# iKrishneel/fcn_object_detector

Measured on AMD Instinct MI355X. Metric: frames/sec forward 448x448 @1 GPU; train imgs/sec @1/2/4/8 GPUs, higher is better.
Workload: dtype f32; 1 GPU; configs[1]: single-GPU forward, DetectNet GoogLeNet conv stack + coverage/bbox heads (graph of models/deploy.prototxt), batch=1, 448x448, random-init weights; global_batch=1, parallelism=replicas x1, frames_in_flight=4

## Files before the change

fcn_object_detector_amd/csrc/conv_fwd.hip:

```cpp
#include <cstddef>
#include <algorithm>
#include <mutex>
#include <unordered_map>
#include <type_traits>

#include "common.h"
#include "conv_common.h"

using namespace fcn;

namespace fcn {

const float* zero_page_for_current_device(int* rc) {
    static std::mutex mu;
    static const float* pages[64] = {nullptr};
    int dev = 0;
    *rc = 0;
    if (hipGetDevice(&dev) != hipSuccess || dev < 0 || dev >= 64) {
        *rc = set_err(FCN_E_STATE, "conv: no current device");
        return nullptr;
    }
    std::lock_guard<std::mutex> lock(mu);
    if (!pages[dev]) {
        void* ptr = nullptr;
        hipError_t e = hipMalloc(&ptr, 256);
        if (e == hipSuccess) e = hipMemset(ptr, 0, 256);
        if (e != hipSuccess) {
            *rc = set_err(-(int)e, "conv: zero page allocation failed: %s", hipGetErrorString(e));
            return nullptr;
        }
        pages[dev] = reinterpret_cast<const float*>(ptr);
    }
    return pages[dev];
}

}

namespace {

constexpr int kPoolItemsPerThread = 2;
constexpr int kPoolSmallItems = 128 * 1024;

template <typename T, int NT>
__device__ __forceinline__ void pool_body(const PoolP& q, int wg) {
    constexpr int EPS = 16 / (int)sizeof(T);
    typedef T vec_t __attribute__((ext_vector_type(EPS)));
    const int cg = q.C / EPS;
    const T* x = reinterpret_cast<const T*>(q.x);
    T* y = reinterpret_cast<T*>(q.y);
    const int ipt = q.items <= kPoolSmallItems ? 1 : kPoolItemsPerThread;
#pragma unroll
    for (int it = 0; it < kPoolItemsPerThread; ++it) {
        if (it >= ipt) return;
        const int t = (wg * ipt + it) * NT + (int)threadIdx.x;
        if (t >= q.items) return;
        const int pix = t / cg;
        const int g = t - pix * cg;
        const int row = pix / q.OW;
        const int ox = pix - row * q.OW;
        const int n = row / q.OH;
        const int oy = row - n * q.OH;
        int hs = oy * q.stride - q.pad, ws = ox * q.stride - q.pad;
        const int he = min(hs + q.k, q.H), we = min(ws + q.k, q.W);
        hs = max(hs, 0);
        ws = max(ws, 0);
        const T* xb = x + (size_t)n * q.H * q.W * q.x_cstride + g * EPS;
        vec_t m;
        int mi[EPS];
#pragma unroll
        for (int e = 0; e < EPS; ++e) {
            m[e] = sizeof(T) == 2 ? (T)-65504.f : (T)-3.402823466e+38f;
            mi[e] = -1;
        }
        if (q.k == 3) {
            const int y0 = oy * q.stride - q.pad, x0 = ox * q.stride - q.pad;
            vec_t v[9];
            int id[9];
            bool in[9];
#pragma unroll
            for (int r = 0; r < 3; ++r) {
                const int iy = min(max(y0 + r, 0), q.H - 1);
#pragma unroll
                for (int c = 0; c < 3; ++c) {
                    const int ix = min(max(x0 + c, 0), q.W - 1);
                    in[3 * r + c] = (int)((unsigned)(y0 + r) < (unsigned)q.H) & (int)((unsigned)(x0 + c) < (unsigned)q.W);
                    id[3 * r + c] = iy * q.W + ix;
                    v[3 * r + c] = *(const vec_t*)(xb + (size_t)id[3 * r + c] * q.x_cstride);
                }
            }
#pragma unroll
// ... 817 lines not shown
    }
#endif
}

__device__ __forceinline__ const GroupArgs& group_of(const GroupArgs& a) { return a; }
__device__ __forceinline__ const GroupArgs& group_of(const GroupArgsTail& a) { return a.g; }
#ifdef FCN_EXP_TAIL_NOLDS
constexpr int kTailLdsFloats = 0;
#else
constexpr int kTailLdsFloats = kTailRows * 32 + 4;
#endif

template <typename T, int WTM, int WTN, int WAVES_M, int WAVES_N, int WAVES_K, int BK, int NBUF, bool PF, bool TAIL = false>
__global__ __launch_bounds__((Cfg<WTM, WTN, WAVES_M, WAVES_N, WAVES_K, BK, NBUF, PF>::NT)) void conv_fwd_group(const int nprob, const int te0, const int te1, const int te2,
                                                                                  const int te3, const int te4, const int te5, const int te6,
                                                                                  const int te7, const int pool_wgs, const int snake,
                                                                                  const std::conditional_t<TAIL, GroupArgsTail, GroupArgs> a_) {
    __shared__ __attribute__((aligned(16))) float smem[Cfg<WTM, WTN, WAVES_M, WAVES_N, WAVES_K, BK, NBUF, PF>::LDS_FLOATS + (TAIL ? kTailLdsFloats : 0)];
    const GroupArgs& a = group_of(a_);
    typedef unsigned u32x16 __attribute__((ext_vector_type(16)));
    typedef unsigned u32x8 __attribute__((ext_vector_type(8)));
    typedef const GroupArgs __attribute__((address_space(4))) * karg_ptr;
    static_assert(alignof(GroupArgsTail) == alignof(GroupArgs) && offsetof(GroupArgsTail, g) == 0, "the group leads its tail");
    constexpr size_t kArgsOffset = (11 * sizeof(int) + alignof(GroupArgs) - 1) / alignof(GroupArgs) * alignof(GroupArgs);
    karg_ptr ka = (karg_ptr)((const char __attribute__((address_space(4)))*)__builtin_amdgcn_kernarg_segment_ptr() + kArgsOffset);
    const int head[1 + kMaxGroup] = {nprob, te0, te1, te2, te3, te4, te5, te6, te7};
    static_assert(kMaxGroup == 8, "the tile prefix travels as eight scalar kernel arguments");
    const int pool_first = pool_wgs > 0 ? pool_wgs : 0;
    if ((int)blockIdx.x < pool_first || (pool_wgs < 0 && (int)blockIdx.x >= te7)) {
        const int w = pool_wgs < 0 ? (int)blockIdx.x - te7 : (int)blockIdx.x;
        if (w < a.pool[0].wg_end) pool_body<T, Cfg<WTM, WTN, WAVES_M, WAVES_N, WAVES_K, BK, NBUF, PF>::NT>(a.pool[0], w);
        else pool_body<T, Cfg<WTM, WTN, WAVES_M, WAVES_N, WAVES_K, BK, NBUF, PF>::NT>(a.pool[1], w - a.pool[0].wg_end);
        return;
    }
    int pos = blockIdx.x;
    if (snake > 0) {
        const int sh = snake & 255, rounds = snake >> 8;
        const int r = pos >> sh, j = pos & ((1 << sh) - 1);
        if (r > 0 && r < rounds - 1 && ((rounds - 1 - r) & 1)) pos = (r << sh) + ((1 << sh) - 1 - j);
    }
    int tile = pos - pool_first;
    if (snake == (int)0x80000000) {
        const int x = pos & 7, sl = pos >> 3, q = te7 >> 3, r = te7 & 7;
        tile = x * q + (x < r ? x : r) + sl;
    } else if (snake < 0) {
        tile += snake;
        tile += tile < 0 ? te7 : 0;
    }
    int pi = 0, begin = 0;
#pragma unroll
    for (int i = 0; i < kMaxGroup - 1; ++i) {
        const int end_i = head[1 + i];
        const bool past = i + 1 < nprob && tile >= end_i;
        pi += past ? 1 : 0;
        begin = past ? end_i : begin;
    }
    u32x16 ra, rb;
    u32x8 rc;
    pi = __builtin_amdgcn_readfirstlane(pi);
    begin = __builtin_amdgcn_readfirstlane(begin);
    const ConvP __attribute__((address_space(4)))* pbase = &ka->p[pi];
    asm volatile("s_load_dwordx16 %0, %3, 0x0\n\ts_load_dwordx16 %1, %3, 0x40\n\ts_load_dwordx8 %2, %3, 0x80\n\ts_waitcnt lgkmcnt(0)"
                 : "=&s"(ra), "=&s"(rb), "=&s"(rc)
                 : "s"(pbase)
                 : "memory");
    ConvP prob;
    __builtin_memcpy((char*)&prob, &ra, 64);
    __builtin_memcpy((char*)&prob + 64, &rb, 64);
    __builtin_memcpy((char*)&prob + 128, &rc, 32);
    if constexpr (TAIL) {
        tail_kptr tp = (tail_kptr)((const char __attribute__((address_space(4)))*)ka + offsetof(GroupArgsTail, tail));
        conv_body<T, WTM, WTN, WAVES_M, WAVES_N, WAVES_K, BK, NBUF, PF, true>(prob, tile - begin, smem, tp);
    } else {
        conv_body<T, WTM, WTN, WAVES_M, WAVES_N, WAVES_K, BK, NBUF, PF>(prob, tile - begin, smem);
    }
}

template <typename T, int WTM, int WTN, int WAVES_M, int WAVES_N, int WAVES_K, int BK, int NBUF, bool PF>
__global__ __launch_bounds__((Cfg<WTM, WTN, WAVES_M, WAVES_N, WAVES_K, BK, NBUF, PF>::NT)) void conv_fwd_one(ConvP p) {
    __shared__ __attribute__((aligned(16))) float smem[Cfg<WTM, WTN, WAVES_M, WAVES_N, WAVES_K, BK, NBUF, PF>::LDS_FLOATS];
    conv_body<T, WTM, WTN, WAVES_M, WAVES_N, WAVES_K, BK, NBUF, PF>(p, blockIdx.x, smem);
}

constexpr int kD7Th = 8, kD7Tw = 32;
constexpr int kD7Ph = 2 * kD7Th + 5, kD7Pw = 2 * kD7Tw + 6;
constexpr int kD7RowF = kD7Pw * 3;
constexpr int kD7PatchF = kD7Ph * kD7RowF;
constexpr int kD7WRowF = 22, kD7WPitchF = 7 * kD7WRowF;
constexpr int kD7WOff = (kD7PatchF + 3) / 4 * 4;
constexpr int kD7EpiPitch = 68;
constexpr int kD7StageF = kD7WOff + 64 * kD7WPitchF;
constexpr int kD7EpiF = 4 * 2 * 32 * kD7EpiPitch;
constexpr int kD7LdsBytes = (kD7StageF > kD7EpiF ? kD7StageF : kD7EpiF) * 4;
constexpr int kD7Threads = 256;
static_assert(kD7LdsBytes <= 80 * 1024, "first-layer kernel: two workgroups per CU");

__global__ __launch_bounds__(kD7Threads) void conv_first7_kernel(const ConvP p) {
#if defined(__HIP_DEVICE_COMPILE__)
    __shared__ __attribute__((aligned(16))) float smem[kD7LdsBytes / 4];
    const int tid = threadIdx.x, lane = tid & 63, wave = __builtin_amdgcn_readfirstlane(tid >> 6);
    FCN_STAMP(0);
    const int tiles_x = (p.OW + kD7Tw - 1) / kD7Tw, tiles_y = (p.OH + kD7Th - 1) / kD7Th;
    int t = blockIdx.x;
    const int tx = t % tiles_x;
    t /= tiles_x;
    const int ty = t % tiles_y, n = t / tiles_y;
    const int oy0 = ty * kD7Th, ox0 = tx * kD7Tw;
    const int iy0 = 2 * oy0 - 3, ix0 = 2 * ox0 - 3;
    const v4f zero4 = {0.f, 0.f, 0.f, 0.f};
    constexpr int PI = (kD7Ph * kD7Pw + kD7Threads - 1) / kD7Threads, WI = (64 * 49 + kD7Threads - 1) / kD7Threads;
    v4f px[PI], wv[WI];
    const float* xn = p.x + (size_t)n * p.H * p.W * 4;
#pragma unroll
    for (int i = 0; i < PI; ++i) {
        const int s = tid + kD7Threads * i;
        const int pr = s / kD7Pw, pc = s - pr * kD7Pw;
        const int iy = iy0 + pr, ix = ix0 + pc;
        const bool ok = s < kD7Ph * kD7Pw && (unsigned)iy < (unsigned)p.H && (unsigned)ix < (unsigned)p.W;
        px[i] = ok ? *reinterpret_cast<const v4f*>(xn + ((size_t)iy * p.W + ix) * 4) : zero4;
    }
#pragma unroll
    for (int i = 0; i < WI; ++i) {
        const int tp = tid + kD7Threads * i;
        wv[i] = tp < p.Cout * 49 ? *reinterpret_cast<const v4f*>(p.w + (size_t)tp * 4) : zero4;
    }
#pragma unroll
    for (int i = 0; i < PI; ++i) {
        const int s = tid + kD7Threads * i;
        if (s < kD7Ph * kD7Pw) {
            float* d = smem + s * 3;
            d[0] = px[i][0]; d[1] = px[i][1]; d[2] = px[i][2];
        }
    }
#pragma unroll
    for (int i = 0; i < WI; ++i) {
        const int tp = tid + kD7Threads * i;
        if (tp < 64 * 49) {
            const int co = tp / 49, rq = tp - co * 49;
            const int r = rq / 7, q = rq - r * 7;
            float* d = smem + kD7WOff + co * kD7WPitchF + r * kD7WRowF + q * 3;
            d[0] = wv[i][0]; d[1] = wv[i][1]; d[2] = wv[i][2];
        }
    }
    for (int i = tid; i < 64 * 7; i += kD7Threads) smem[kD7WOff + i * kD7WRowF + 21] = 0.f;
    const int c4 = (lane & 15) * 4;
    const v4f bias_v = (p.bias && c4 < p.Cout) ? *reinterpret_cast<const v4f*>(p.bias + c4) : zero4;
    FCN_STAMP(1);
    const int nl = lane & 31, h = lane >> 5;
    const float* a_base = smem + (4 * wave) * kD7RowF + 6 * nl + h;
    const float* b_base = smem + kD7WOff + nl * kD7WPitchF + h;
    typedef float v16f __attribute__((ext_vector_type(16)));
    v16f acc[2][2];
#pragma unroll
    for (int i = 0; i < 2; ++i)
#pragma unroll
        for (int j = 0; j < 2; ++j)
#pragma unroll
            for (int e = 0; e < 16; ++e) acc[i][j][e] = 0.f;
    __syncthreads();
    FCN_STAMP(2);
    auto frag = [&](const int step, float (&a)[2], float (&b)[2]) {
        const int r = step / 11, j = step - 11 * r;
#pragma unroll
        for (int mt = 0; mt < 2; ++mt) a[mt] = a_base[(2 * mt + r) * kD7RowF + 2 * j];
#pragma unroll
        for (int nt = 0; nt < 2; ++nt) b[nt] = b_base[nt * 32 * kD7WPitchF + r * kD7WRowF + 2 * j];
    };
    float fa[3][2], fb[3][2];
    frag(0, fa[0], fb[0]);
    frag(1, fa[1], fb[1]);
#pragma unroll
    for (int step = 0; step < 77; ++step) {
        if (step + 2 < 77) frag(step + 2, fa[(step + 2) % 3], fb[(step + 2) % 3]);
        __builtin_amdgcn_sched_barrier(0);
#pragma unroll
        for (int mt = 0; mt < 2; ++mt)
#pragma unroll
            for (int nt = 0; nt < 2; ++nt)
                acc[mt][nt] = __builtin_amdgcn_mfma_f32_32x32x2f32(fa[step % 3][mt], fb[step % 3][nt], acc[mt][nt], 0, 0, 0);
    }
    FCN_STAMP(3);
    __syncthreads();
    float* epi = smem + wave * (2 * 32 * kD7EpiPitch);
#pragma unroll
    for (int mt = 0; mt < 2; ++mt)
#pragma unroll
        for (int nt = 0; nt < 2; ++nt)
#pragma unroll
            for (int v = 0; v < 16; ++v) epi[(mt * 32 + (v & 3) + 8 * (v >> 2) + 4 * h) * kD7EpiPitch + nl + 32 * nt] = acc[mt][nt][v];
    asm volatile("s_waitcnt lgkmcnt(0)" ::: "memory");
    __builtin_amdgcn_sched_barrier(0);
    const bool do_relu = (p.flags & FCN_CONV_RELU) != 0;
#pragma unroll
    for (int mt = 0; mt < 2; ++mt) {
        const int oy = oy0 + 2 * wave + mt;
        float* yrow = p.y + ((size_t)(n * p.OH + oy) * p.OW + ox0) * p.y_cstride + p.y_coffset + c4;
#pragma unroll
        for (int i = 0; i < 8; ++i) {
            const int ox = (lane >> 4) + 4 * i;
            v4f v = *reinterpret_cast<const v4f*>(epi + (mt * 32 + ox) * kD7EpiPitch + c4) + bias_v;
            if (do_relu)
#pragma unroll
                for (int e = 0; e < 4; ++e) v[e] = fmaxf(v[e], 0.f);
            if (oy < p.OH && ox0 + ox < p.OW && c4 < p.Cout) *reinterpret_cast<v4f*>(yrow + (size_t)ox * p.y_cstride) = v;
        }
    }
#ifdef FCN_CONV_STAMPS
    FCN_STAMP(5);
    wait_vmcnt<0>();
    FCN_STAMP(6);
#endif
#endif
}

constexpr int kH7PatchSlots = (kD7Ph * kD7Pw + 63) / 64 * 64;
constexpr int kH7EpiOff = 2 * kH7PatchSlots * 16;
constexpr int kH7EpiPitch = 144;
constexpr int kH7LdsBytes = kH7EpiOff + 4 * 64 * kH7EpiPitch;
static_assert(kH7LdsBytes <= 160 * 1024, "half-float first-layer kernel: LDS image");

__global__ __launch_bounds__(kD7Threads) void conv_first7_f16_kernel(const ConvP p, const int ntiles) {
#if defined(__HIP_DEVICE_COMPILE__)
    __shared__ __attribute__((aligned(16))) char smem[kH7LdsBytes];
    const int tid = threadIdx.x, lane = tid & 63, wave = __builtin_amdgcn_readfirstlane(tid >> 6);
    const int tiles_x = (p.OW + kD7Tw - 1) / kD7Tw, tiles_y = (p.OH + kD7Th - 1) / kD7Th;
    const f16_t* xh = reinterpret_cast<const f16_t*>(p.x);
    const f16_t* wh = reinterpret_cast<const f16_t*>(p.w);
    f16_t* yh = reinterpret_cast<f16_t*>(p.y);
    const v4f zero4 = {0.f, 0.f, 0.f, 0.f};
    constexpr int PI = (kD7Ph * kD7Pw + kD7Threads - 1) / kD7Threads;
    auto fetch_patch = [&](const int tile, v4f (&px)[PI]) {
        int t = tile;
        const int tx = t % tiles_x;
        t /= tiles_x;
        const int ty = t % tiles_y, n = t / tiles_y;
        const int iy0 = 2 * ty * kD7Th - 3, ix0 = 2 * tx * kD7Tw - 3;
        const f16_t* xn = xh + (size_t)n * p.H * p.W * 8;
#pragma unroll
        for (int i = 0; i < PI; ++i) {
            const int s = tid + kD7Threads * i;
            const int pr = s / kD7Pw, pc = s - pr * kD7Pw;
            const int iy = iy0 + pr, ix = ix0 + pc;
            const bool ok = tile < ntiles && s < kD7Ph * kD7Pw && (unsigned)iy < (unsigned)p.H && (unsigned)ix < (unsigned)p.W;
            px[i] = ok ? *reinterpret_cast<const v4f*>(xn + ((size_t)iy * p.W + ix) * 8) : zero4;
        }
    };
    auto store_patch = [&](const int buf, const v4f (&px)[PI]) {
#pragma unroll
        for (int i = 0; i < PI; ++i) {
            const int s = tid + kD7Threads * i;
            if (s < kD7Ph * kD7Pw) *reinterpret_cast<v4f*>(smem + (buf * kH7PatchSlots + s) * 16) = px[i];
        }
    };
    const int nl = lane & 31, h = lane >> 5;
    v4f px[PI];
    int tile = blockIdx.x;
    fetch_patch(tile, px);
    v4f breg[28][2];
#pragma unroll
    for (int step = 0; step < 28; ++step)
#pragma unroll
        for (int nt = 0; nt < 2; ++nt) {
            const int r = step >> 2, q = (step & 3) + 4 * h, co = 2 * nl + nt;
// ... 1019 lines not shown
```

fcn_object_detector_amd/csrc/pointwise.hip:

```cpp
#include <float.h>
#include <math.h>

#include "common.h"

using namespace fcn;

namespace {

__device__ __forceinline__ float4 ld4(const float* p) { return *reinterpret_cast<const float4*>(p); }
__device__ __forceinline__ void st4(float* p, float4 v) { *reinterpret_cast<float4*>(p) = v; }

template <typename D>
__global__ __launch_bounds__(256) void nchw_to_nhwc_kernel(const float* __restrict__ src, D* __restrict__ dst,
                                                           int C, int HW, int dst_cstride, int dst_coffset, float shift) {
    __shared__ float tile[32][33];
    const int n = blockIdx.z;
    const int p0 = blockIdx.x * 32, c0 = blockIdx.y * 32;
    const int tx = threadIdx.x & 31, ty = threadIdx.x >> 5;
    const float* s = src + (size_t)n * C * HW;
    D* d = dst + (size_t)n * HW * dst_cstride;
    for (int i = ty; i < 32; i += 8) {
        const int c = c0 + i, p = p0 + tx;
        tile[i][tx] = (c < C && p < HW) ? s[(size_t)c * HW + p] : 0.f;
    }
    __syncthreads();
    for (int i = ty; i < 32; i += 8) {
        const int p = p0 + i, c = c0 + tx;
        if (p < HW && c < C) d[(size_t)p * dst_cstride + dst_coffset + c] = (D)(tile[tx][i] + shift);
    }
}

template <typename S>
__global__ __launch_bounds__(256) void nhwc_to_nchw_kernel(const S* __restrict__ src, float* __restrict__ dst,
                                                           int C, int HW, int src_cstride, int src_coffset) {
    __shared__ float tile[32][33];
    const int n = blockIdx.z;
    const int p0 = blockIdx.x * 32, c0 = blockIdx.y * 32;
    const int tx = threadIdx.x & 31, ty = threadIdx.x >> 5;
    const S* s = src + (size_t)n * HW * src_cstride;
    float* d = dst + (size_t)n * C * HW;
    for (int i = ty; i < 32; i += 8) {
        const int p = p0 + i, c = c0 + tx;
        tile[i][tx] = (p < HW && c < C) ? (float)s[(size_t)p * src_cstride + src_coffset + c] : 0.f;
    }
    __syncthreads();
    for (int i = ty; i < 32; i += 8) {
        const int c = c0 + i, p = p0 + tx;
        if (c < C && p < HW) d[(size_t)c * HW + p] = tile[tx][i];
    }
}

__global__ __launch_bounds__(256) void nchw_to_nhwc4_kernel(const float* __restrict__ src, float* __restrict__ dst, int C, int HW, float shift) {
    const int n = blockIdx.y;
    const float* s = src + (size_t)n * C * HW;
    for (int p = blockIdx.x * blockDim.x + threadIdx.x; p < HW; p += gridDim.x * blockDim.x) {
        float4 v = make_float4(0.f, 0.f, 0.f, 0.f);
        v.x = s[p] + shift;
        if (C > 1) v.y = s[(size_t)HW + p] + shift;
        if (C > 2) v.z = s[2 * (size_t)HW + p] + shift;
        if (C > 3) v.w = s[3 * (size_t)HW + p] + shift;
        *reinterpret_cast<float4*>(dst + ((size_t)n * HW + p) * 4) = v;
    }
}

constexpr int kMaxLayoutBlobs = 8;
struct LayoutBlob { const float* src; float* dst; int C, HW, cstride, coffset, count, end; };
struct LayoutArgs { int n; LayoutBlob b[kMaxLayoutBlobs]; };
__global__ __launch_bounds__(256) void nhwc_to_nchw_multi_kernel(const LayoutArgs a) {
    const int total = a.b[a.n - 1].end;
    for (int i = blockIdx.x * blockDim.x + threadIdx.x; i < total; i += gridDim.x * blockDim.x) {
        int k = 0;
#pragma unroll
        for (int j = 0; j < kMaxLayoutBlobs - 1; ++j) k += (j + 1 < a.n && i >= a.b[j].end) ? 1 : 0;
        LayoutBlob q = a.b[0];
#pragma unroll
        for (int j = 1; j < kMaxLayoutBlobs; ++j)
            if (k == j) q = a.b[j];
        const int e = i - (q.end - q.count);
        const int p = e % q.HW, nc = e / q.HW;
        const int c = nc % q.C, n = nc / q.C;
        q.dst[e] = q.src[((size_t)n * q.HW + p) * q.cstride + q.coffset + c];
    }
}

template <bool VEC4, bool WITH_IDX>
__global__ __launch_bounds__(256) void maxpool_kernel(const float* __restrict__ x, float* __restrict__ y, int32_t* __restrict__ idx,
                                                      int N, int H, int W, int C, int x_cstride, int k, int stride, int pad,
                                                      int OH, int OW, int y_cstride, int y_coffset) {
    const int cg = VEC4 ? C / 4 : C;
    const long long total = (long long)N * OH * OW * cg;
    for (long long t = (long long)blockIdx.x * blockDim.x + threadIdx.x; t < total; t += (long long)gridDim.x * blockDim.x) {
        const int g = (int)(t % cg);
        long long pix = t / cg;
// ... 5 lines not shown
        const int he = min(hs + k, H), we = min(ws + k, W);
        hs = max(hs, 0);
        ws = max(ws, 0);
        const float* xb = x + (size_t)n * H * W * x_cstride + (VEC4 ? g * 4 : g);
        const size_t o = ((size_t)(n * OH + oy) * OW + ox);
        if (VEC4) {
            float4 m = make_float4(-FLT_MAX, -FLT_MAX, -FLT_MAX, -FLT_MAX);
            int4 mi = make_int4(-1, -1, -1, -1);
            if (k == 3) {
                const int y0 = oy * stride - pad, x0 = ox * stride - pad;
                float4 v[9];
                int id[9];
                bool in[9];
#pragma unroll
                for (int r = 0; r < 3; ++r) {
                    const int iy = min(max(y0 + r, 0), H - 1);
#pragma unroll
                    for (int c = 0; c < 3; ++c) {
                        const int ix = min(max(x0 + c, 0), W - 1);
                        in[3 * r + c] = (unsigned)(y0 + r) < (unsigned)H && (unsigned)(x0 + c) < (unsigned)W;
                        id[3 * r + c] = iy * W + ix;
                        v[3 * r + c] = ld4(xb + (size_t)id[3 * r + c] * x_cstride);
                    }
                }
#pragma unroll
                for (int t9 = 0; t9 < 9; ++t9) {
                    if (in[t9] & (v[t9].x > m.x)) { m.x = v[t9].x; mi.x = id[t9]; }
                    if (in[t9] & (v[t9].y > m.y)) { m.y = v[t9].y; mi.y = id[t9]; }
                    if (in[t9] & (v[t9].z > m.z)) { m.z = v[t9].z; mi.z = id[t9]; }
                    if (in[t9] & (v[t9].w > m.w)) { m.w = v[t9].w; mi.w = id[t9]; }
                }
            } else
            for (int iy = hs; iy < he; ++iy)
                for (int ix = ws; ix < we; ++ix) {
                    const float4 v = ld4(xb + ((size_t)iy * W + ix) * x_cstride);
                    const int id = iy * W + ix;
                    if (v.x > m.x) { m.x = v.x; mi.x = id; }
                    if (v.y > m.y) { m.y = v.y; mi.y = id; }
                    if (v.z > m.z) { m.z = v.z; mi.z = id; }
                    if (v.w > m.w) { m.w = v.w; mi.w = id; }
                }
            st4(y + o * y_cstride + y_coffset + g * 4, m);
            if (WITH_IDX) *reinterpret_cast<int4*>(idx + o * C + g * 4) = mi;
        } else {
            float m = -FLT_MAX;
            int mi = -1;
            for (int iy = hs; iy < he; ++iy)
                for (int ix = ws; ix < we; ++ix) {
                    const float v = xb[((size_t)iy * W + ix) * x_cstride];
                    if (v > m) { m = v; mi = iy * W + ix; }
                }
            y[o * y_cstride + y_coffset + g] = m;
            if (WITH_IDX) idx[o * C + g] = mi;
        }
    }
}

__global__ __launch_bounds__(256) void avepool_kernel(const float* __restrict__ x, float* __restrict__ y, int N, int H, int W, int C,
                                                      int x_cstride, int k, int stride, int pad, int OH, int OW, int y_cstride,
                                                      int y_coffset) {
    const long long total = (long long)N * OH * OW * C;
    for (long long t = (long long)blockIdx.x * blockDim.x + threadIdx.x; t < total; t += (long long)gridDim.x * blockDim.x) {
        const int c = (int)(t % C);
        long long pix = t / C;
        const int ox = (int)(pix % OW);
        pix /= OW;
        const int oy = (int)(pix % OH);
        const int n = (int)(pix / OH);
        int hs = oy * stride - pad, ws = ox * stride - pad;
        int he = min(hs + k, H + pad), we = min(ws + k, W + pad);
        const float area = (float)((he - hs) * (we - ws));
        hs = max(hs, 0);
        ws = max(ws, 0);
        he = min(he, H);
        we = min(we, W);
        const float* xb = x + (size_t)n * H * W * x_cstride + c;
        float acc = 0.f;
        for (int iy = hs; iy < he; ++iy)
            for (int ix = ws; ix < we; ++ix) acc += xb[((size_t)iy * W + ix) * x_cstride];
        y[((size_t)(n * OH + oy) * OW + ox) * y_cstride + y_coffset + c] = acc / area;
    }
}

__device__ __forceinline__ float pow_neg_beta(float s, float beta) {
    if (beta == 0.75f) {
        const float r = sqrtf(s);
        return 1.f / (r * sqrtf(r));
    }
    return powf(s, -beta);
}

__device__ __forceinline__ float pow_neg_beta_fast(float s, float beta) {
    if (beta == 0.75f) {
        const float r = __builtin_amdgcn_rsqf(s);
        return r * __builtin_amdgcn_sqrtf(r);
    }
    return powf(s, -beta);
}

template <bool FAST = false>
__device__ __forceinline__ float4 lrn5_apply(const float4 l, const float4 c, const float4 r, float alpha_over_n, float beta, float kk, float4& s) {
    const float q[12] = {l.x * l.x, l.y * l.y, l.z * l.z, l.w * l.w, c.x * c.x, c.y * c.y,
                         c.z * c.z, c.w * c.w, r.x * r.x, r.y * r.y, r.z * r.z, r.w * r.w};
    s.x = kk + alpha_over_n * (q[2] + q[3] + q[4] + q[5] + q[6]);
    s.y = kk + alpha_over_n * (q[3] + q[4] + q[5] + q[6] + q[7]);
    s.z = kk + alpha_over_n * (q[4] + q[5] + q[6] + q[7] + q[8]);
    s.w = kk + alpha_over_n * (q[5] + q[6] + q[7] + q[8] + q[9]);
    float4 o;
    o.x = c.x * (FAST ? pow_neg_beta_fast(s.x, beta) : pow_neg_beta(s.x, beta));
    o.y = c.y * (FAST ? pow_neg_beta_fast(s.y, beta) : pow_neg_beta(s.y, beta));
    o.z = c.z * (FAST ? pow_neg_beta_fast(s.z, beta) : pow_neg_beta(s.z, beta));
    o.w = c.w * (FAST ? pow_neg_beta_fast(s.w, beta) : pow_neg_beta(s.w, beta));
    return o;
}

__global__ __launch_bounds__(256) void lrn5_kernel(const float* __restrict__ x, float* __restrict__ y, float* __restrict__ scale,
                                                   long long pixels, int C, int x_cstride, int y_cstride, float alpha_over_n,
                                                   float beta, float kk) {
    const int cg = C / 4;
    const long long total = pixels * cg;
    for (long long t = (long long)blockIdx.x * blockDim.x + threadIdx.x; t < total; t += (long long)gridDim.x * blockDim.x) {
        const int g = (int)(t % cg);
        const long long pix = t / cg;
        const float* xp = x + (size_t)pix * x_cstride + g * 4;
        const float4 c = ld4(xp);
        const float4 l = g > 0 ? ld4(xp - 4) : make_float4(0.f, 0.f, 0.f, 0.f);
        const float4 r = g + 1 < cg ? ld4(xp + 4) : make_float4(0.f, 0.f, 0.f, 0.f);
        float4 s;
        const float4 o = lrn5_apply(l, c, r, alpha_over_n, beta, kk, s);
        st4(y + (size_t)pix * y_cstride + g * 4, o);
        if (scale) st4(scale + (size_t)pix * C + g * 4, s);
    }
}

__device__ __forceinline__ float4 max4(const float4 a, const float4 b) {
    return make_float4(b.x > a.x ? b.x : a.x, b.y > a.y ? b.y : a.y, b.z > a.z ? b.z : a.z, b.w > a.w ? b.w : a.w);
}

template <bool LRN_FIRST>
__global__ __launch_bounds__(512) void maxpool_lrn5_kernel(const float* __restrict__ x, float* __restrict__ y, int H, int W, int C, int x_cstride,
                                                           int k, int stride, int pad, int OH, int OW, int y_cstride, int cgroups,
                                                           float alpha_over_n, float beta, float kk) {
    const int cg32 = (int)blockIdx.x % cgroups, tx = (int)blockIdx.x / cgroups;
    const int g = cg32 * 8 + ((int)threadIdx.x & 7), cg = C / 4;
    const int pp = (int)threadIdx.x >> 3;
    const int oy = (int)blockIdx.y * 8 + (pp >> 3), ox = tx * 8 + (pp & 7), n = (int)blockIdx.z;
    if (g >= cg || oy >= OH || ox >= OW) return;
    int hs = oy * stride - pad, ws = ox * stride - pad;
    const int he = min(hs + k, H), we = min(ws + k, W);
    hs = max(hs, 0);
    ws = max(ws, 0);
    const float* xb = x + (size_t)n * H * W * x_cstride + g * 4;
    const bool hl = g > 0, hr = g + 1 < cg;
    const float4 zero = make_float4(0.f, 0.f, 0.f, 0.f), low = make_float4(-FLT_MAX, -FLT_MAX, -FLT_MAX, -FLT_MAX);
    float4 m = low, ml = hl ? low : zero, mr = hr ? low : zero, s;
    for (int iy = hs; iy < he; ++iy)
        for (int ix = ws; ix < we; ++ix) {
            const float* xp = xb + ((size_t)iy * W + ix) * x_cstride;
            const float4 c = ld4(xp);
            const float4 l = hl ? ld4(xp - 4) : zero;
            const float4 r = hr ? ld4(xp + 4) : zero;
            if (LRN_FIRST) {
                m = max4(m, lrn5_apply<true>(l, c, r, alpha_over_n, beta, kk, s));
            } else {
                m = max4(m, c);
                if (hl) ml = max4(ml, l);
                if (hr) mr = max4(mr, r);
            }
        }
    if (!LRN_FIRST) m = lrn5_apply(ml, m, mr, alpha_over_n, beta, kk, s);
    st4(y + ((size_t)(n * OH + oy) * OW + ox) * y_cstride + g * 4, m);
}

constexpr int kPLC_C = 64, kPLC_Pitch = 68;
__global__ __launch_bounds__(256) void pool3_lrn5_conv1x1_kernel(const float* __restrict__ x, const float* __restrict__ w, const float* __restrict__ bias,
                                                                 float* __restrict__ y, int H, int W, int x_cstride, int stride, int pad, int OH, int OW,
                                                                 int y_cstride, int y_coffset, int relu, float alpha_over_n, float beta, float kk) {
    __shared__ __attribute__((aligned(16))) float act[32 * kPLC_Pitch];
    const int tid = threadIdx.x, lane = tid & 63, wave = tid >> 6;
    const int n = (int)blockIdx.z;
    const int fi = lane & 15, fh = lane >> 4;
    const float* wp = w + (size_t)(16 * wave + fi) * kPLC_C + 16 * fh;
    float4 wf[4];
#pragma unroll
    for (int j = 0; j < 4; ++j) wf[j] = ld4(wp + 4 * j);
    const float4 bv = bias ? ld4(bias + 16 * wave + 4 * fh) : make_float4(0.f, 0.f, 0.f, 0.f);
    const int p = tid >> 3, q = tid & 7;
    const int oy = min((int)blockIdx.y * 4 + (p >> 3), OH - 1), ox = min((int)blockIdx.x * 8 + (p & 7), OW - 1);
    const int hs = oy * stride - pad, ws = ox * stride - pad;
    const int h0 = max(hs, 0), h1 = min(hs + 3, H) - 1, w0 = max(ws, 0), w1 = min(ws + 3, W) - 1;
    const float* xb = x + (size_t)n * H * W * x_cstride + 8 * q;
    float4 t0[9], t1[9];
#pragma unroll
    for (int r = 0; r < 3; ++r)
#pragma unroll
        for (int c = 0; c < 3; ++c) {
            const int iy = min(max(hs + r, h0), h1), ix = min(max(ws + c, w0), w1);
            const float* xp = xb + ((size_t)iy * W + ix) * x_cstride;
            t0[3 * r + c] = ld4(xp);
            t1[3 * r + c] = ld4(xp + 4);
        }
    float4 m0 = t0[0], m1 = t1[0];
#pragma unroll
    for (int i = 1; i < 9; ++i) {
        m0 = max4(m0, t0[i]);
        m1 = max4(m1, t1[i]);
    }
    float4 lft, rgt;
    lft.x = __shfl_up(m1.x, 1); lft.y = __shfl_up(m1.y, 1); lft.z = __shfl_up(m1.z, 1); lft.w = __shfl_up(m1.w, 1);
    rgt.x = __shfl_down(m0.x, 1); rgt.y = __shfl_down(m0.y, 1); rgt.z = __shfl_down(m0.z, 1); rgt.w = __shfl_down(m0.w, 1);
    const float4 zero = make_float4(0.f, 0.f, 0.f, 0.f);
    if (q == 0) lft = zero;
    if (q == 7) rgt = zero;
    float4 s;
    const float4 a0 = lrn5_apply<true>(lft, m0, m1, alpha_over_n, beta, kk, s);
    const float4 a1 = lrn5_apply<true>(m0, m1, rgt, alpha_over_n, beta, kk, s);
    st4(act + p * kPLC_Pitch + 8 * q, a0);
    st4(act + p * kPLC_Pitch + 8 * q + 4, a1);
    __syncthreads();
// ... 1401 lines not shown
```

fcn_object_detector_amd/detector.py:

```python
from __future__ import annotations

import ctypes as C
import os
import math
from typing import Dict, List, Optional, Sequence, Tuple

import numpy as np

from . import lib as L
from .engine import DeviceBuffer, Engine, PinnedArray, replica_streams

F32 = np.float32


class HeadMapping:

    def __init__(self, cvg_blob: str, bbox_blob: str, stride: int, skip_background: bool):
        self.cvg_blob, self.bbox_blob, self.stride, self.skip_background = cvg_blob, bbox_blob, int(stride), bool(skip_background)

    @classmethod
    def reference_node(cls) -> "HeadMapping":
        return cls("pool_score", "upscore_pool5_bbox", 8, True)

    @classmethod
# ... 188 lines not shown
        boxes[i, 0] = boxes[i, 0] * diffx
        boxes[i, 1] = boxes[i, 1] * diffy
        boxes[i, 2] = boxes[i, 2] * diffx
        boxes[i, 3] = boxes[i, 3] * diffy
    return boxes


def detection_window_roi(im_shape: Sequence[int], stride: int = 2) -> np.ndarray:
    im_y, im_x = int(im_shape[0]), int(im_shape[1])
    stride = int(stride)
    if stride < 1 or im_x < stride or im_y < stride:
        raise ValueError("detection_window_roi: stride %d does not divide a %d x %d frame into windows" % (stride, im_x, im_y))
    w, h = im_x // stride, im_y // stride
    rects = [(i * w, j * h, w, h) for j in range(stride) for i in range(stride)]
    rects.append((im_x // 2 - w // 2, im_y // 2 - h // 2, w, h))
    return np.asarray(rects, dtype=np.int32)


class FCNObjectDetector:

    def __init__(self, engine: Engine, detection_threshold: float = 0.5, min_boxes: int = 3, nms_eps: float = 0.2,
                 mapping: Optional[HeadMapping] = None, round_mode: int = L.RECT_ROUND_NEAREST_EVEN):
        self.engine = engine
        self.prob_thresh, self.min_boxes, self.eps = detection_threshold, min_boxes, nms_eps
        self.mapping = mapping or HeadMapping.auto(list(engine.blobs))
        data = engine.blobs["data"]
        self.batch, _, self.im_height, self.im_width = data.shape
        cvg, box = engine.blobs[self.mapping.cvg_blob], engine.blobs[self.mapping.bbox_blob]
        skip = 1 if self.mapping.skip_background else 0
        self.num_classes = cvg.channels - skip
        gx, gy = int(self.im_width / self.mapping.stride), int(self.im_height / self.mapping.stride)
        if (gy, gx) != tuple(cvg.shape[2:]):
            raise ValueError("grid %dx%d from stride %d does not match blob %s %s" % (gy, gx, self.mapping.stride,
                                                                                     self.mapping.cvg_blob, cvg.shape))
        self.decoder = GridDecoder(self.batch, self.num_classes, gy, gx, self.im_width, self.im_height, self.prob_thresh,
                                   self.min_boxes, self.eps, 20, round_mode)
        self._cvg_args = (cvg.buf.ptr, cvg.cstride, cvg.coffset + skip, cvg.pixels // self.batch * cvg.cstride)
        self._box_args = (box.buf.ptr, box.cstride, box.coffset, box.pixels // self.batch * box.cstride)
        self._frame_dev: Optional[DeviceBuffer] = None
        self._minmax = DeviceBuffer(32)
        self._minmax_batch_holder: List[DeviceBuffer] = []

    def _half_flag(self, data) -> int:
        if data.esize != 2:
            return 0
        return 3 if data.name in self.engine._half_inputs and data.cstride == 8 and data.coffset == 0 else 1

    def run_detector_batch(self, frames: Sequence[np.ndarray]) -> List[Tuple[np.ndarray, np.ndarray]]:
        self.submit_batch(frames)
        return self.collect_batch()

    def submit_batch(self, frames: Sequence[np.ndarray]) -> None:
        eng = self.engine
        if len(frames) != self.batch:
            raise ValueError("need %d frames (the engine's batch), got %d" % (self.batch, len(frames)))
        if getattr(self, "_outstanding", None) is not None:
            raise RuntimeError("a batch is already in flight: collect_batch() it first")
        frames = [np.ascontiguousarray(f, np.uint8) for f in frames]
        if any(f.ndim != 3 or f.shape[2] != 3 for f in frames):
            raise ValueError("expected BGR uint8 frames")
        with eng.lock:
            L.call("fcn_init", eng.device)
            need = sum((f.nbytes + 15) // 16 * 16 for f in frames)
            if self._frame_dev is None or self._frame_dev.nbytes < need:
                self._frame_dev = DeviceBuffer(need, zero=False)
                self._frame_pinned = PinnedArray(((need + 3) // 4,))
            stage = self._frame_pinned.array.view(np.uint8)
            data = eng.blobs["data"]
            if len(self._minmax_batch_holder) == 0 or self._minmax_batch_holder[0].nbytes < 32 * len(frames):
                self._minmax_batch_holder[:] = [DeviceBuffer(32 * len(frames))]
            same = all(f.shape == frames[0].shape for f in frames)
            off, offs = 0, []
            for f in frames:
                stage[off:off + f.nbytes] = f.reshape(-1)
                offs.append(off)
                off += f.nbytes if same else (f.nbytes + 15) // 16 * 16
            L.call("fcn_memcpy_h2d_async", self._frame_dev.ptr, stage.ctypes.data, off, eng.stream)
            self._enqueue_batch(self._frame_dev.ptr, [(o, f.shape[0], f.shape[1]) for o, f in zip(offs, frames)], same)
            self._outstanding = [f.shape for f in frames]

    def _enqueue_batch(self, dev_ptr: int, layout: Sequence[Tuple[int, int, int]], same: bool) -> None:
        eng = self.engine
        data = eng.blobs["data"]
        if same:
            L.call("fcn_preprocess_bgr8_batch", dev_ptr, len(layout), layout[0][1], layout[0][2], data.ptr, self._half_flag(data),
                   self.im_height, self.im_width, data.cstride, data.upload_shift, self._minmax_batch_holder[0].ptr, eng.stream)
        else:
            for i, (off, h, w) in enumerate(layout):
                L.call("fcn_preprocess_bgr8_batch", dev_ptr + off, 1, h, w, data.ptr + data.esize * i * self.im_height * self.im_width * data.cstride,
                       self._half_flag(data), self.im_height, self.im_width, data.cstride, data.upload_shift, self._minmax.ptr, eng.stream)
        eng.forward_enqueue()
        self.decoder.launch(*self._cvg_args, *self._box_args, eng.stream)
        self.decoder.fetch_begin(eng.stream)
        data.host_valid = False

    def run_detector2(self, frame: np.ndarray, stride: int = 2) -> Tuple[np.ndarray, List[Tuple[np.ndarray, np.ndarray]]]:
        eng = self.engine
        frame = np.ascontiguousarray(frame, np.uint8)
        if frame.ndim != 3 or frame.shape[2] != 3:
            raise ValueError("expected a BGR uint8 frame")
        rects = detection_window_roi(frame.shape, stride)
        if len(rects) != self.batch:
            raise ValueError("stride %d makes %d windows; the engine's batch is %d" % (stride, len(rects), self.batch))
        if getattr(self, "_outstanding", None) is not None:
            raise RuntimeError("a batch is already in flight: collect it first")
        h, w, _c = frame.shape
        with eng.lock:
            L.call("fcn_init", eng.device)
            if self._frame_dev is None or self._frame_dev.nbytes < frame.nbytes:
                self._frame_dev = DeviceBuffer(frame.nbytes, zero=False)
                self._frame_pinned = PinnedArray(((frame.nbytes + 3) // 4,))
            stage = self._frame_pinned.array.view(np.uint8)[:frame.nbytes]
            stage[...] = frame.reshape(-1)
            data = eng.blobs["data"]
            L.call("fcn_memcpy_h2d_async", self._frame_dev.ptr, stage.ctypes.data, frame.nbytes, eng.stream)
            L.call("fcn_preprocess_bgr8_rois", self._frame_dev.ptr, h, w, rects.ctypes.data, len(rects), data.ptr, self._half_flag(data),
                   self.im_height, self.im_width, data.cstride, data.upload_shift, self._minmax.ptr, eng.stream)
            eng.forward_enqueue()
            self.decoder.launch(*self._cvg_args, *self._box_args, eng.stream)
            self.decoder.fetch_begin(eng.stream)
            data.host_valid = False
            res = self.decoder.fetch(eng.stream, begun=True)
        out = []
        for (x, y, rw, rh), (dets, labels) in zip(rects.tolist(), res):
            boxes = np.asarray(dets, dtype=np.int64).reshape(-1, 5)
            if len(boxes):
                boxes = resize_detection((rh, rw), boxes, self.im_width, self.im_height)
                boxes[:, 0] += x; boxes[:, 2] += x
                boxes[:, 1] += y; boxes[:, 3] += y
            out.append((boxes, labels))
        return rects, out

    def run_detector2_masks(self, frame: np.ndarray, stride: int = 1, score_blob: str = "score", padding: int = 10):
        eng = self.engine
        frame = np.ascontiguousarray(frame, np.uint8)
        if frame.ndim != 3 or frame.shape[2] != 3:
            raise ValueError("expected a BGR uint8 frame")
        rects = detection_window_roi(frame.shape, stride)
        if len(rects) != self.batch:
            raise ValueError("stride %d makes %d windows; the engine's batch is %d" % (stride, len(rects), self.batch))
        sb = eng.blobs[score_blob]
        if sb.esize != 4 or len(sb.shape) != 4:
            raise NotImplementedError("score blob %s must be a 4-d float32 blob" % score_blob)
        h, w, _c = frame.shape
        _n, C_, sh, sw = sb.shape
        key = (len(rects), C_, int(rects[0][2]), int(rects[0][3]), h, w)
        if getattr(self, "_score_masks_key", None) != key:
            self._score_masks = ScoreMasks(*key)
            self._score_masks_key = key
        with eng.lock:
            L.call("fcn_init", eng.device)
            if self._frame_dev is None or self._frame_dev.nbytes < frame.nbytes:
                self._frame_dev = DeviceBuffer(frame.nbytes, zero=False)
                self._frame_pinned = PinnedArray(((frame.nbytes + 3) // 4,))
            stage = self._frame_pinned.array.view(np.uint8)[:frame.nbytes]
            stage[...] = frame.reshape(-1)
            data = eng.blobs["data"]
            L.call("fcn_memcpy_h2d_async", self._frame_dev.ptr, stage.ctypes.data, frame.nbytes, eng.stream)
            L.call("fcn_preprocess_bgr8_rois", self._frame_dev.ptr, h, w, rects.ctypes.data, len(rects), data.ptr, self._half_flag(data),
                   self.im_height, self.im_width, data.cstride, data.upload_shift, self._minmax.ptr, eng.stream)
            eng.forward_enqueue()
            for op in eng._lazy_blob_ops.get(score_blob, ()):
                op.run(eng.stream)
            self._score_masks.launch(sb.buf.ptr, sh, sw, sb.cstride, sb.coffset, rects, self.prob_thresh, eng.stream)
            data.host_valid = False
            return self._score_masks.fetch(eng.stream, padding)

    def collect_batch(self) -> List[Tuple[np.ndarray, np.ndarray]]:
        if getattr(self, "_outstanding", None) is None:
            raise RuntimeError("no batch in flight")
        shapes, self._outstanding = self._outstanding, None
        with self.engine.lock:
            res = self.decoder.fetch(self.engine.stream, begun=True)
        out = []
        for shape, (dets, labels) in zip(shapes, res):
            boxes = np.asarray(dets, dtype=np.int64).reshape(-1, 5)
            out.append((resize_detection(shape, boxes, self.im_width, self.im_height) if len(boxes) else boxes, labels))
        return out

    def submit(self, frame: np.ndarray) -> None:
        eng = self.engine
        if self.batch != 1:
            raise ValueError("run_detector handles one frame; build the engine with batch 1")
        if getattr(self, "_outstanding", None) is not None:
            raise RuntimeError("a frame is already in flight: collect() it first")
        frame = np.ascontiguousarray(frame, np.uint8)
        if frame.ndim != 3 or frame.shape[2] != 3:
            raise ValueError("expected a BGR uint8 frame")
        h, w, _c = frame.shape
        with eng.lock:
            L.call("fcn_init", eng.device)
            if self._frame_dev is None or self._frame_dev.nbytes < frame.nbytes:
                self._frame_dev = DeviceBuffer(frame.nbytes, zero=False)
                self._frame_pinned = PinnedArray(((frame.nbytes + 3) // 4,))
            stage = self._frame_pinned.array.view(np.uint8)[:frame.nbytes]
            stage[...] = frame.reshape(-1)
            data = eng.blobs["data"]
            L.call("fcn_memcpy_h2d_async", self._frame_dev.ptr, stage.ctypes.data, frame.nbytes, eng.stream)
            L.call("fcn_preprocess_bgr8_batch", self._frame_dev.ptr, 1, h, w, data.ptr, self._half_flag(data), self.im_height, self.im_width,
                   data.cstride, data.upload_shift, self._minmax.ptr, eng.stream)
            eng.forward_enqueue()
            self.decoder.launch(*self._cvg_args, *self._box_args, eng.stream)
            self.decoder.fetch_begin(eng.stream)
            data.host_valid = False
            self._outstanding = frame.shape

    def collect(self) -> Tuple[np.ndarray, np.ndarray]:
        if getattr(self, "_outstanding", None) is None:
            raise RuntimeError("no frame in flight")
        shape, self._outstanding = self._outstanding, None
        with self.engine.lock:
            dets, labels = self.decoder.fetch(self.engine.stream, begun=True)[0]
        boxes = np.asarray(dets, dtype=np.int64).reshape(-1, 5)
        if not len(boxes):
            return boxes, labels
        return resize_detection(shape, boxes, self.im_width, self.im_height), labels

    def run_detector(self, frame: np.ndarray) -> Tuple[np.ndarray, np.ndarray]:
        self.submit(frame)
        return self.collect()


class DetectorPipeline:

    def __init__(self, make_engine, depth: int = 3, **detector_kw):
        self.detectors: List[FCNObjectDetector] = []
        first = None
        with replica_streams():
            for _ in range(max(int(depth), 1)):
                eng = make_engine(first)
                first = first or eng
                self.detectors.append(FCNObjectDetector(eng, **detector_kw))
        self._queue: List[FCNObjectDetector] = []
        self._next = 0

    def submit(self, frame: np.ndarray) -> None:
        if len(self._queue) >= len(self.detectors):
            raise RuntimeError("DetectorPipeline: %d frames already in flight" % len(self._queue))
        d = self.detectors[self._next]
        self._next = (self._next + 1) % len(self.detectors)
        d.submit(frame)
        self._queue.append(d)

    def collect(self) -> Tuple[np.ndarray, np.ndarray]:
        if not self._queue:
            raise RuntimeError("DetectorPipeline: nothing in flight")
        return self._queue.pop(0).collect()

    def run_detector_batches(self, batches) -> List[List[Tuple[np.ndarray, np.ndarray]]]:
        out, queue, nxt = [], [], 0
        for frames in batches:
            if len(queue) == len(self.detectors):
                out.append(queue.pop(0).collect_batch())
            d = self.detectors[nxt]
            nxt = (nxt + 1) % len(self.detectors)
            d.submit_batch(frames)
            queue.append(d)
        while queue:
            out.append(queue.pop(0).collect_batch())
        return out

    def run_detector_stream(self, frames) -> List[Tuple[np.ndarray, np.ndarray]]:
        out = []
        for f in frames:
            if len(self._queue) == len(self.detectors):
                out.append(self.collect())
            self.submit(f)
        while self._queue:
            out.append(self.collect())
        return out

    def close(self) -> None:
        for d in self.detectors:
            d.engine.close()
```

fcn_object_detector_amd/engine.py:

```python
from __future__ import annotations

import ctypes as C
import os
import threading
from collections import namedtuple
from dataclasses import dataclass, field
from typing import Callable, Dict, List, Optional, Sequence, Tuple, Union

import numpy as np

from . import lib as L
from . import region as RG
from . import ssd as SSD
from . import storage as S
from . import tune as T
from .netspec import (ACT_TYPES, Layer, NetSpec, argmax_form, bn_global_stats, crop_window, interp_size, is_rectangular, is_scale_gate, kernel_stride_pad,
                      layer_dilation, layer_geometry, scale_gate_form)
from .storage import _r4, _ra, ip_pack_bank, ip_unpack_bank

F32 = np.float32


def graphs_enabled() -> bool:
    return os.environ.get("FCN_NO_GRAPH", "0") in ("", "0")
# ... 199 lines not shown
    def contiguous(self) -> bool:
        return self.coffset == 0 and self.cstride == self.channels


class Op:

    def __init__(self, kind: str, name: str, run: Callable[[Optional[int]], None], flops: float = 0.0, bytes_: float = 0.0):
        self.kind = kind
        self.name = name
        self.run = run
        self.flops = flops
        self.bytes = bytes_


Range = Tuple[int, int, int]


@dataclass(eq=False)
class ConvTask:
    layer: Layer
    desc: L.ConvDesc
    flops: float
    bytes: float
    reads: List[Range]
    writes: List[Range]


@dataclass(eq=False)
class OpTask:
    layer: Layer
    ops: List[Op]
    reads: List[Range]
    writes: List[Range]
    pool_desc: Optional[L.PoolDesc] = None
    rconv: Optional[L.RConvDesc] = None
    dwconv: Optional[L.DwConvDesc] = None


Task = Union[ConvTask, OpTask]


@dataclass(eq=False)
class BnChain:
    x: str
    y: str
    bn: Optional[Layer] = None
    scale: Optional[Layer] = None
    relu: Optional[Layer] = None
    mids: List[str] = field(default_factory=list)
    save: Optional["DeviceBuffer"] = None
    global_stats: bool = False


@dataclass(eq=False)
class ArgChain:
    x: str
    y: str
    argmax: Optional[Layer] = None
    interp: Optional[Layer] = None
    softmax: Optional[Layer] = None
    mids: List[str] = field(default_factory=list)


def ranges_hit(a: Sequence[Range], b: Sequence[Range]) -> bool:
    return any(x[0] == y[0] and x[1] < y[2] and y[1] < x[2] for x in a for y in b)


def task_waits(later: Task, earlier: Task) -> bool:
    return ranges_hit(later.reads, earlier.writes) or ranges_hit(later.writes, earlier.writes) or ranges_hit(later.writes, earlier.reads)


def task_levels(tasks: Sequence[Task], group_convs: bool = True) -> List[int]:
    levels: List[int] = []
    for i, ti in enumerate(tasks):
        levels.append(max([levels[j] + 1 for j in range(i) if task_waits(ti, tasks[j])], default=0) if group_convs else i)
    return levels


def task_floats(tasks: Sequence[Task], levels: Sequence[int], i: int) -> bool:
    return not any(levels[j] == levels[i] + 1 and task_waits(tj, tasks[i]) for j, tj in enumerate(tasks) if j != i)


class Engine:

    def __init__(self, spec: NetSpec, data_shapes: Optional[Dict[str, Tuple[int, ...]]] = None,
                 params: Optional[Dict[str, List[np.ndarray]]] = None, device: int = 0,
                 fuse: bool = True, group_convs: bool = True, autotune: bool = True, dtype: str = "f32",
                 tune_from: Optional["Engine"] = None, tune_max_lds_kb: Optional[int] = None,
                 share_params: Optional["Engine"] = None, score_outputs: bool = False, replica: Optional[int] = None):
        if dtype not in ("f32", "f16"):
            raise ValueError("dtype must be 'f32' or 'f16'")
        if share_params is not None and (dtype != "f32" or share_params.f16):
            raise NotImplementedError("share_params: only between float32 engines (a half-float engine packs its weights differently)")
        self._share_from = share_params
        self.shared_layers: set = set()
        self.score_outputs = bool(score_outputs)
        self.score_acc: Dict[str, DeviceBuffer] = {}
        self.graph_score: Optional[int] = None
        if dtype == "f16" and spec.phase != "TEST":
            raise NotImplementedError("the half-float path is inference only (BASELINE configs[4])")
        self.dtype, self.f16 = dtype, dtype == "f16"
        self.spec = spec
        self.device = device
        self.fuse = fuse
        self.group_convs = group_convs
        self.autotune = autotune
        L.call("fcn_init", device)
        sp = C.c_void_p()
        self.replica = replica if replica is not None else _take_replica_index()
        if self.replica is None:
            L.call("fcn_stream_create", C.byref(sp))
        else:
            L.call("fcn_stream_create_replica", C.byref(sp), int(self.replica))
        self.stream = int(sp.value)
        yes = C.c_int(0)
        L.call("fcn_stream_is_prioritized", self.stream, C.byref(yes))
        self.stream_prioritized = bool(yes.value)
        self.lock = threading.RLock()
        self.shapes = spec.infer(data_shapes)
        self.blobs: Dict[str, Blob] = {}
        self.params_host: Dict[str, List[np.ndarray]] = {}
        self.params_dev: Dict[str, List[DevView]] = {}
        self.ops: List[Op] = []
        self.graph_io: Optional[int] = None
        self.graph_core: Optional[int] = None
        self._staging: Dict[str, DeviceBuffer] = {}
        self._keep: List[object] = []
        self._conv_layer_meta: Dict[str, dict] = {}
        self._group_workspaces: List[DeviceBuffer] = []
        self.aux_dev: Dict[str, DeviceBuffer] = {}
        self._bn_chains: Dict[str, BnChain] = {}
        self._bn_ws_bytes = 0
        self._bn_ws: Optional[DeviceBuffer] = None
        self._lazy_blob_ops: Dict[str, List[Op]] = {}
        self.loss_blobs: Dict[str, float] = {}
        self.device_fed: set = set()
        self.dropout_seed = 0
        self.dropout_index_offset = 0
        self.inputs = spec.data_tops()
        self.outputs = [b for b in spec.output_blobs() if b in self.shapes and b not in spec.mask_blobs]
        max_lds = int(tune_max_lds_kb if tune_max_lds_kb is not None else os.environ.get("FCN_TUNE_MAX_LDS_KB", "160")) * 1024
        self.tuner = T.Tuner(self.stream, T.key_suffix(self.shapes.get(self.inputs[0], ()) if self.inputs else None, self.f16, max_lds),
                             spec.phase == "TEST", max_lds, tune_from._chosen_cfgs if tune_from is not None else None)
        self._plan_buffers()
        self._alloc_params(params)
        self._build_ops()
        self.tuner.release()

    @property
    def _chosen_cfgs(self) -> Dict[str, object]:
        return self.tuner.chosen

    def _plan_buffers(self) -> None:
        plan = S.plan_blobs(self.spec, self.shapes, self.inputs, self.outputs, self.f16, self.fuse, os.environ.get("FCN_F16_IMAGE", "1") != "0")
        self.producers, self.consumers = plan.producers, plan.consumers
        self.alias, self.shift, self.copy_concats, self.copy_slices = plan.alias, plan.shift, plan.copy_concats, plan.copy_slices
        self._half_inputs = plan.half_inputs
        self.permutes, self.gathers, self.detections = plan.permutes, plan.gathers, plan.detections
        self.pair_softmax, self.rpn_views = plan.pair_softmax, plan.rpn_views
        self.roi_counts: Dict[str, DeviceBuffer] = {}
        self._roi_count_host: Dict[str, "PinnedArray"] = {}
        self._roi_caps: Dict[str, int] = {}
        self._counts_valid = False
        bufs = {root: DeviceBuffer(nbytes) for root, nbytes in plan.root_bytes.items()}
        for name, v in plan.views.items():
            b = self.blobs[name] = Blob(name, v.shape)
            b.esize, b.rows, b.is_input = v.esize, v.rows, name in self.inputs
            b.buf, b.coffset, b.cstride = bufs[v.root], v.coffset, v.cstride
            b.upload_shift, b.lazy_shift = v.upload_shift, v.lazy_shift
        self._upload_priors()
        for d in self._half_inputs:
            b = self.blobs[d]
            ones = np.zeros((b.pixels, b.cstride), np.float16)
            ones[:, 3:5] = 1.0
            L.call("fcn_memcpy_h2d_async", b.buf.ptr, ones.ctypes.data, ones.nbytes, None)
            L.call("fcn_device_sync")

    def _upload_priors(self) -> None:
        self.prior_consts: Dict[str, np.ndarray] = {}
        for name, l in self.spec.prior_blobs.items():
            if l.type == "PriorBox":
                _, _, fh, fw = self.shapes[l.bottoms[0]]
                _, _, dh, dw = self.shapes[l.bottoms[1]]
                a = SSD.prior_boxes(SSD.priorbox_params(l), fh, fw, dh, dw)
            else:
                a = np.concatenate([self.prior_consts[b] for b in l.bottoms], axis=2)
            if a.shape != tuple(self.shapes[name]):
                raise RuntimeError("layer %s: %s prior constants for the blob %s" % (l.name, a.shape, self.shapes[name]))
            self.prior_consts[name] = a = np.ascontiguousarray(a, F32)
            b = self.blobs[name]
            if b.coffset or b.cstride != a.size:
                raise NotImplementedError("layer %s: the prior blob %s is a window of another buffer" % (l.name, name))
            L.call("fcn_memcpy_h2d_async", b.buf.ptr, a.ctypes.data, a.nbytes, None)
            L.call("fcn_device_sync")

    def _alloc_params(self, params: Optional[Dict[str, List[np.ndarray]]]) -> None:
        from .netspec import fill_params
        if params is None:
            params = fill_params(self.spec, seed=0)
        self.param_segs: Dict[Tuple[str, int], S.ParamSeg] = {}
        src = self._share_from
        if src is not None:
            self._shared_keep = [src.param_flat] + list(getattr(src, "_shared_keep", []))
            for l in self.spec.param_layers():
                if l.name not in src.params_dev:
                    continue
                mine, theirs = [tuple(x) for x in self.spec.param_shapes[l.name]], [tuple(x) for x in src.spec.param_shapes[l.name]]
                if mine != theirs:
                    raise ValueError("share_params: layer %s has blobs %s here and %s in the source net" % (l.name, mine, theirs))
                self.shared_layers.add(l.name)
                self.params_host[l.name] = src.params_host[l.name]
                self.params_dev[l.name] = [DevView(v.ptr, v.nbytes) for v in src.params_dev[l.name]]
                self.param_segs.update({(l.name, i): src.param_segs[(l.name, i)] for i in range(len(mine))})
        self.param_layout, self.param_count = S.param_layout(self.spec, self.blobs, self.f16, self.shared_layers)
        for l in self.spec.param_layers():
            if l.name in self.shared_layers:
                continue
# ... 319 lines not shown
        spec = self.spec
        skip: set = set()
        tasks: List[Task] = []
        self._conv_flags: Dict[str, int] = {}
        self._gate_fused: Dict[str, Layer] = {}
        for li, l in enumerate(spec.layers):
            if l.name in skip:
                continue
            t = l.type
            if t in ("Data", "Python", "Input", "DummyData", "MemoryData", "ImageData", "HDF5Data"):
                continue
            if spec.is_depthwise(l):
                tasks.append(self._dwconv_task(li, l, skip))
                continue
            if t == "Convolution" and (is_rectangular(l) or layer_dilation(l) > 1):
                tasks.append(self._rconv_task(li, l, skip))
                continue
            if t == "Convolution":
                top = l.tops[0]
                fused_relu, sig_top = self._fused_after(li, l, skip)
                g, ng = self._geom(l), self._conv_groups(l)
                cin_g, cout_g = g.cin // ng, g.cout // ng
                (xp, xlo, _), (yp, ylo, _) = self._range(l.bottoms[0]), self._range(top)
                for i in range(ng):
                    tasks.append(ConvTask(l, self._conv_desc(l, fused_relu, sig_top, i), g.flops / (ng * ng),
                                          4.0 * (g.n * cin_g * g.h * g.w + g.n * cout_g * g.oh * g.ow + cout_g * cin_g * g.k * g.k + cout_g),
                                          reads=[(xp, xlo + i * cin_g, xlo + (i + 1) * cin_g)],
                                          writes=[(yp, ylo + i * cout_g, ylo + (i + 1) * cout_g)] + ([self._range(sig_top)] if sig_top else [])))
                self._conv_layer_meta[l.name] = dict(relu=fused_relu, sigmoid_top=sig_top)
                self._conv_flags[l.name] = int(tasks[-1].desc.flags)
                continue
            if t == "InnerProduct":
                relu = self._relu_after(li, l, skip)
                self._conv_layer_meta[l.name] = dict(relu=relu, sigmoid_top=None)
                tasks.append(OpTask(l, self._fwd_inner_product(l, relu), reads=[self._range(l.bottoms[0])], writes=[self._range(l.tops[0])]))
                continue
            if is_scale_gate(l):
                if self._gate_fusion(li, l) is None:
                    tasks.append(OpTask(l, [self._scale_gate_op(l, None, None)], reads=[self._range(b) for b in l.bottoms], writes=[self._range(l.tops[0])]))
                continue
            if t == "Eltwise" and l.name in self._gate_fused:
                sc, before = self._gate_fused[l.name], set(skip)
                relu = next(iter(skip - before)) if self._relu_after(li, l, skip) else None
                self._lazy_blob_ops[sc.tops[0]] = [self._scale_gate_op(sc, None, None)]
                tasks.append(OpTask(l, [self._scale_gate_op(sc, l, relu)], reads=[self._range(b) for b in sc.bottoms + [self._gate_residual(sc, l)]],
                                    writes=[self._range(l.tops[0])]))
                continue
            if t in ("BatchNorm", "Scale"):
                ch = self._bn_chain_after(li, l, skip)
                tasks.append(OpTask(l, self._fwd_batchnorm(ch), reads=[self._range(ch.x)], writes=[self._range(ch.y)]))
                continue
            if t in RG.REGION_TYPES or l.name in self.pair_softmax or (t == "Reshape" and (l.tops[0] in self.rpn_views or l.bottoms[0] in self.rpn_views)):
                tasks.extend(self._region_tasks(l))
                continue
            if t in SSD.HEAD_TYPES or l.name in self.gathers or (l.tops and l.tops[0] in spec.prior_blobs) or \
                    (t == "Softmax" and len(self.shapes[l.bottoms[0]]) == 3 and int(l.sub("softmax_param").get("axis", 1)) in (2, -1)):
                tasks.extend(self._ssd_tasks(l))
                continue
            if t == "Concat" and l.name not in self.copy_concats:
                continue
            if t == "Slice" and l.name not in self.copy_slices:
                continue
            if t == "Dropout" and spec.phase == "TEST" and (l.tops[0] == l.bottoms[0] or l.tops[0] in self.alias):
                continue
            if t == "Power" and l.tops[0] in self.shift:
                continue
            if t in ("Interp", "Softmax", "ArgMax"):
                ch = self._argmax_chain_at(l, skip)
                if ch is not None:
                    tasks.append(OpTask(ch.argmax, self._fwd_argmax(ch), reads=[self._range(ch.x)], writes=[self._range(ch.y)]))
                    continue
            ops = self._emit_simple(l)
            read = l.bottoms[:1] if t == "Crop" else l.bottoms
            tasks.append(OpTask(l, ops, reads=[self._range(b) for b in read], writes=[self._range(tp) for tp in l.tops],
                                pool_desc=self._fusable_pool_desc(l)))
        return tasks

    def _build_ops(self) -> None:
        tasks = self._collect_tasks()
        if self._bn_ws_bytes:
            self._bn_ws = DeviceBuffer(self._bn_ws_bytes, zero=False)
        if self.fuse and self.spec.phase == "TEST" and os.environ.get("FCN_FUSE_POOL_LRN", "1") != "0":
            tasks = self._fuse_pool_lrn(tasks)
        levels = task_levels(tasks, self.group_convs)
        if self.autotune and self.group_convs and self.fuse and not self.f16 and self.spec.phase == "TEST" and os.environ.get("FCN_LEVEL_MOVE", "1") != "0":
            self.tuner.move_floaters(tasks, levels)
        tail = self._plan_tail(tasks, levels)
        order = sorted(range(len(tasks)), key=lambda i: (levels[i], 1 if isinstance(tasks[i], ConvTask) else 0, i))
        pending: List[ConvTask] = []
        pending_pools: List[OpTask] = []
        pending_rconvs: List[OpTask] = []
        cur = None
        for i in order:
            if levels[i] != cur:
                self._emit_rconvs(pending_rconvs)
                self._emit_convs(pending, pending_pools, tail)
                pending, pending_rconvs, cur = [], [], levels[i]
            if tail is not None and any(tasks[i] is ht for ht in tail["heads"]):
                continue
            if isinstance(tasks[i], ConvTask):
                pending.append(tasks[i])
            elif tasks[i].pool_desc is not None and self.fuse and self.group_convs:
                pending_pools.append(tasks[i])
            elif tasks[i].rconv is not None:
                pending_rconvs.append(tasks[i])
            else:
                self.ops.extend(tasks[i].ops)
        self._emit_rconvs(pending_rconvs)
        self._emit_convs(pending, pending_pools, tail)
        self.levels = max(levels) + 1 if levels else 0
        if self.score_outputs:
            self._emit_score_ops()

    def _ssd_tasks(self, l: Layer) -> List[OpTask]:
        lib, B, t = L.load(), self.blobs, l.type
        need = getattr(self, "need_grad", None)
        if need is not None and any(b in need for b in l.bottoms + l.tops):
            raise NotImplementedError("layer %s: %s below a layer that learns in a TRAIN-phase net (the SSD head has no backward pass: "
                                      "deploy nets only)" % (l.name, t))
        if l.name in self.gathers:
            top, cols = self.gathers[l.name]
            db = B[top]
            n, width = db.shape[0], db.shape[1]
            out: List[OpTask] = []
            for g0 in range(0, len(cols), L.SSD_MAX_HEADS):
                part = cols[g0:g0 + L.SSD_MAX_HEADS]
                arr = (L.SsdHead * len(part))()
                byts = 0.0
                for h, (_flat, src, col) in zip(arr, part):
                    sb = B[src]
                    if sb.esize != 4 or sb.nchw is None or sb.shape[0] != n:
                        raise NotImplementedError("layer %s: the head %s is no float32 4-d blob of %d images" % (l.name, src, n))
                    h.src, h.pixels, h.C, h.cstride, h.coffset, h.dst_col = sb.buf.ptr, sb.shape[2] * sb.shape[3], sb.shape[1], sb.cstride, sb.coffset, col
                    byts += 8.0 * n * h.pixels * h.C
                self._keep.append(arr)
                label = l.name + ":" + "+".join(src for _f, src, _c in part)
                run = lambda st, arr=arr, k=len(part): L.check(lib.fcn_ssd_gather_f32(arr, k, n, db.buf.ptr + 4 * db.coffset, db.cstride, width, st))
                out.append(OpTask(l, [Op("ssd_gather", label, run, 0.0, byts)], reads=[self._range(src) for _f, src, _c in part],
                                  writes=[(db.buf.ptr, db.coffset + part[0][2], db.coffset + part[-1][2] + B[part[-1][0]].channels)]))
            return out
        if t in ("Permute", "Reshape", "Flatten", "PriorBox") or (t == "Concat" and l.tops[0] in self.spec.prior_blobs):
            return []
        if t == "Normalize":
            xb, yb = B[l.bottoms[0]], B[l.tops[0]]
            npar = l.sub("norm_param")
            shared, eps = int(bool(npar.get("channel_shared", True))), float(npar.get("eps", 1e-10))
            scale = self.params_dev[l.name][0]
            if yb.cstride < yb.coffset + _r4(yb.channels):
                raise NotImplementedError("layer %s: the top %s is a channel window that ends inside a 16-byte group" % (l.name, l.tops[0]))
            pix, c = xb.pixels, xb.channels
            run = lambda st: L.check(lib.fcn_normalize_fwd_f32(xb.buf.ptr, yb.buf.ptr, scale.ptr, pix, c, xb.cstride, xb.coffset, yb.cstride,
                                                               yb.coffset, shared, eps, st))
            return [OpTask(l, [Op("normalize", l.name, run, 4.0 * pix * c, 8.0 * pix * c)], reads=[self._range(l.bottoms[0])],
                           writes=[self._range(l.tops[0])])]
        if t == "Softmax":
            xb, yb = B[l.bottoms[0]], B[l.tops[0]]
            if len(xb.shape) != 3 or not xb.rows or xb.shape != yb.shape:
                raise NotImplementedError("Softmax over an axis other than channels (layer %s)" % l.name)
            n, pr, c = xb.shape
            def run(st):
                for i in range(n):
                    L.check(lib.fcn_softmax_fwd_f32(xb.ptr + 4 * i * xb.cstride, yb.ptr + 4 * i * yb.cstride, pr, c, c, c, st))
            return [OpTask(l, [Op("softmax", l.name, run, 0.0, 8.0 * n * pr * c)], reads=[self._range(l.bottoms[0])], writes=[self._range(l.tops[0])])]
        if t == "DetectionOutput":
            dp = SSD.detection_params(l)
            (_, _, cap, _), priors = SSD.detection_shapes(l, [self.shapes[b] for b in l.bottoms])
# ... 248 lines not shown
            self.ops.append(Op("score", "score:" + nm, lambda st, a=args: L.check(lib.fcn_score_accumulate_f32(*a, st)), 0.0, 12.0 * count))

    def _plan_tail(self, tasks: List[Task], levels: List[int]) -> Optional[dict]:
        if self.f16 or self.spec.phase != "TEST" or not (self.fuse and self.group_convs) or os.environ.get("FCN_CONV_TAIL", "0") != "1":
            return None
        conv_idx = [i for i, t in enumerate(tasks) if isinstance(t, ConvTask)]
        if not conv_idx:
            return None
        lh = max(levels[i] for i in conv_idx)
        heads = [i for i in conv_idx if levels[i] == lh]
        if any(levels[i] >= lh for i, t in enumerate(tasks) if not isinstance(t, ConvTask)) or not 1 <= len(heads) <= 4:
            return None
        d0 = tasks[heads[0]].desc
        m = d0.N * d0.OH * d0.OW
        rows = 0
        for i in heads:
            d = tasks[i].desc
            if (d.kh, d.kw, d.stride, d.pad) != (1, 1, 1, 0) or d.x != d0.x or d.x_cstride != d0.x_cstride or d.Cin != d0.Cin or d.Cin % 32 or d.Cin > 1024 or d.Cout % 4 \
                    or (d.flags & ~(L.CONV_RELU | L.CONV_SIGMOID2)) or d.y_cstride % 4 or d.y_coffset % 4 or (d.y2 and (d.y2_cstride % 4 or d.y2_coffset % 4)):
                return None
            rows += d.Cout
        if rows > 24 or m > 4096:
            return None
        xr = tasks[heads[0]].reads
        producers: Dict[int, int] = {}
        covered = 0
        for i, t in enumerate(tasks):
            if i in heads or not ranges_hit(t.writes, xr):
                continue
            if not isinstance(t, ConvTask):
                return None
            d = t.desc
            if levels[i] not in (lh - 1, lh - 2) or d.y != d0.x or d.y_cstride != d0.x_cstride or d.N * d.OH * d.OW != m \
                    or d.Cout % 32 or d.y_coffset % 32 or d.y_coffset + d.Cout > d0.Cin or (d.flags & ~L.CONV_RELU) or d.y_cstride % 4:
                return None
            producers[id(t)] = levels[i]
            covered += d.Cout
        if covered != d0.Cin or not producers:
            return None
        for lv in set(producers.values()):
            if sum(1 for i in conv_idx if levels[i] == lv) > 8:
                return None
        lib = L.load()
        desc = L.ConvTail()
        desc.n = len(heads)
        for j, i in enumerate(heads):
            desc.heads[j] = tasks[i].desc
        sb, ab = int(lib.fcn_conv2d_tail_scratch_bytes(C.byref(desc))), int(lib.fcn_conv2d_tail_arrive_bytes(C.byref(desc)))
        if sb <= 0 or ab <= 0:
            return None
        scratch, arrive = DeviceBuffer(sb, zero=False), DeviceBuffer(ab, zero=True)
        desc.scratch, desc.arrive = scratch.ptr, arrive.ptr
        self._keep.extend([scratch, arrive, desc])
        return dict(desc=desc, heads=[tasks[i] for i in heads], producers=producers, final_level=max(producers.values()))

    def _fuse_pool_lrn(self, tasks: List[Task]) -> List[Task]:
        B, lib = self.blobs, L.load()
        out: List[Task] = []
        i = 0
        while i < len(tasks):
            a = tasks[i]
            b = tasks[i + 1] if i + 1 < len(tasks) else None
            op = None
            if isinstance(a, OpTask) and isinstance(b, OpTask):
                la, lb = a.layer, b.layer
                if {la.type, lb.type} == {"Pooling", "LRN"} and len(la.tops) == 1 and lb.bottoms == [la.tops[0]] and la.tops[0] != la.bottoms[0]:
                    op = self._pool_lrn_op(la, lb)
            if op is None:
                out.append(a)
                i += 1
                continue
            self._lazy_blob_ops[a.layer.tops[0]] = list(a.ops)
            c = tasks[i + 2] if i + 2 < len(tasks) else None
            op3 = self._pool_lrn_conv_op(a.layer, b.layer, c) if isinstance(c, ConvTask) else None
            if op3 is not None:
                self._lazy_blob_ops[b.layer.tops[0]] = [op]
                out.append(OpTask(c.layer, [op3], reads=a.reads, writes=c.writes))
                i += 3
                continue
            out.append(OpTask(b.layer, [op], reads=a.reads, writes=b.writes))
            i += 2
        return out

    def _pool_lrn_conv_op(self, la: Layer, lb: Layer, ct: ConvTask) -> Optional[Op]:
        if os.environ.get("FCN_FUSE_POOL_LRN_CONV", "1") == "0" or la.type != "Pooling":
            return None
        B, lib = self.blobs, L.load()
        lc, d = ct.layer, ct.desc
        mid = lb.tops[0]
        if lc.bottoms != [mid] or [q.name for q in self.consumers.get(mid, [])] != [lc.name] or len(self.producers.get(mid, [])) != 1 \
                or mid in self.outputs or mid in self.alias:
            return None
        xb, nb = B[la.bottoms[0]], B[mid]
        k, s, pad = kernel_stride_pad(la.sub("pooling_param"))
        lp = lb.sub("lrn_param")
        esz = xb.esize
        want = (L.CONV_F16 if esz == 2 else 0)
        if (d.kh, d.kw, d.stride, d.pad) != (1, 1, 1, 0) or d.Cin != 64 or d.Cout != 64 or xb.channels != 64 or k != 3 or nb.esize != esz \
                or (d.flags & ~L.CONV_RELU) != want or d.in_shift != 0.0 or nb.coffset or d.y_cstride % (16 // esz) or d.y_coffset % (16 // esz) or B[lc.tops[0]].esize != esz:
            return None
        n, c, h, w = xb.shape
        oh, ow = d.OH, d.OW
        if (oh + 3) // 4 > 65535 or n > 65535:
            return None
        if esz == 2 and ((s, pad) != (2, 0) or n * c * h * w < 1 << 22):
            return None
        al, be, kk = float(lp.get("alpha", 1.0)), float(lp.get("beta", 0.75)), float(lp.get("k", 1.0))
        relu = 1 if d.flags & L.CONV_RELU else 0
        fn = lib.fcn_maxpool_lrn5_conv1x1_fwd_f16 if esz == 2 else lib.fcn_maxpool_lrn5_conv1x1_fwd_f32
        return Op("pool_lrn_conv", "%s+%s+%s" % (la.name, lb.name, lc.name), lambda st: L.check(fn(
            xb.ptr, n, h, w, c, xb.cstride, k, s, pad, oh, ow, al, be, kk, d.w, d.bias, d.Cout, relu, d.y, d.y_cstride, d.y_coffset, st)),
            ct.flops, float(esz) * (xb.pixels * c + n * oh * ow * d.Cout))

    def _pool_lrn_op(self, la: Layer, lb: Layer) -> Optional[Op]:
        B, lib = self.blobs, L.load()
        pool, lrn = (la, lb) if la.type == "Pooling" else (lb, la)
        if len(pool.tops) != 1:
            return None
        mid = la.tops[0]
        if [q.name for q in self.consumers.get(mid, [])] != [lb.name] or len(self.producers.get(mid, [])) != 1 or mid in self.outputs:
            return None
        pp, lp = pool.sub("pooling_param"), lrn.sub("lrn_param")
        if str(pp.get("pool", "MAX")) != "MAX" or bool(pp.get("global_pooling", False)):
            return None
        if str(lp.get("norm_region", "ACROSS_CHANNELS")) != "ACROSS_CHANNELS" or int(lp.get("local_size", 5)) != 5:
            return None
        xb, mb, yb = B[la.bottoms[0]], B[mid], B[lb.tops[0]]
        esz = xb.esize
        eps = 16 // esz
        if any(t.esize != esz or t.coffset or t.cstride % eps for t in (xb, mb, yb)) or xb.channels % eps or mid in self.alias or lb.tops[0] in self.alias:
            return None
        n, c, h, w = xb.shape
        _, _, oh, ow = yb.shape
        k, s, pad = kernel_stride_pad(pp)
        if pad >= k or max((h + 7) // 8, n) > 65535:
            return None
        if n * c * h * w > 8 << 20 and not (esz == 2 and (k, s, pad) == (3, 2, 0) and c <= 192):
            return None
        al, be, kk = float(lp.get("alpha", 1.0)), float(lp.get("beta", 0.75)), float(lp.get("k", 1.0))
        first = 1 if la.type == "LRN" else 0
        fn = lib.fcn_maxpool_lrn5_fwd_f16 if esz == 2 else lib.fcn_maxpool_lrn5_fwd_f32
        return Op("pool_lrn", "%s+%s" % (la.name, lb.name), lambda st: L.check(fn(
            xb.ptr, yb.ptr, n, h, w, c, xb.cstride, k, s, pad, oh, ow, yb.cstride, first, al, be, kk, st)),
            0.0, float(esz) * (xb.pixels * c + yb.pixels * c))

    def _fusable_pool_desc(self, l: Layer) -> Optional[L.PoolDesc]:
        if os.environ.get("FCN_FUSE_POOLS", "1") == "0":
            return None
        xb = self.blobs.get(l.bottoms[0])
        if self.f16 and xb is not None and xb.pixels >= 16384:
            return None
        if self.f16 and len(l.tops) == 2:
            return None
        return self._fusable_pool_desc_impl(l)

    def _fusable_pool_desc_impl(self, l: Layer) -> Optional[L.PoolDesc]:
        if l.type != "Pooling":
            return None
        pp = l.sub("pooling_param")
        if str(pp.get("pool", "MAX")) != "MAX" or bool(pp.get("global_pooling", False)):
            return None
        xb, yb = self.blobs[l.bottoms[0]], self.blobs[l.tops[0]]
        n, c, h, w = xb.shape
        _, _, oh, ow = yb.shape
        k, s, pad = kernel_stride_pad(pp)
        eps = 16 // xb.esize
        if xb.esize != yb.esize or (xb.esize == 2 and self.spec.phase != "TEST"):
            return None
        if c % eps or xb.cstride % eps or yb.cstride % eps or yb.coffset % eps or xb.coffset % eps or n * oh * ow * (c // eps) >= 1 << 30:
            return None
        idx = self.aux_dev.get(l.name)
        d = L.PoolDesc()
        d.x, d.y, d.idx = xb.ptr, yb.buf.ptr, (idx.ptr if idx is not None else None)
        d.N, d.H, d.W, d.C, d.x_cstride, d.k, d.stride, d.pad = n, h, w, c, xb.cstride, k, s, pad
        d.OH, d.OW, d.y_cstride, d.y_coffset = oh, ow, yb.cstride, yb.coffset
        d.f16 = 1 if xb.esize == 2 else 0
        return d

    def _loss_grad_ptr(self, blob: str) -> Optional[int]:
        return None

    def _emit_simple(self, l: Layer) -> List[Op]:
        B, t = self.blobs, l.type
        halves = [b for b in list(l.bottoms) + list(l.tops) if b in B and B[b].esize == 2]
        acts = ACT_TYPES if self.spec.activations else ()
        if halves and t not in ("Pooling", "LRN", "Eltwise", "Softmax", "Deconvolution", "Dropout", "Concat", "Slice", "Crop", "ReLU", "Interp", "Upsample") + acts:
            raise NotImplementedError("f16 engine: layer type %s (%s) has no half-float kernel" % (t, l.name))
        if t in acts:
            return self._fwd_act(l, halves)
        emit = {"Pooling": self._fwd_pooling, "LRN": self._fwd_lrn, "ReLU": self._fwd_pointwise, "Sigmoid": self._fwd_pointwise,
                "Power": self._fwd_pointwise, "Dropout": self._fwd_dropout, "L1Loss": self._fwd_loss, "EuclideanLoss": self._fwd_loss,
                "Softmax": self._fwd_softmax, "SoftmaxWithLoss": self._fwd_softmax_loss, "Accuracy": self._fwd_accuracy,
                "Slice": self._fwd_slice, "Concat": self._fwd_concat, "Eltwise": self._fwd_eltwise,
                "Deconvolution": self._fwd_deconvolution, "Crop": self._fwd_crop, "Interp": self._fwd_interp,
                "Upsample": self._fwd_upsample}.get(t)
# ... 300 lines not shown
        nbytes = int(lib.fcn_ip_gemm_workspace_bytes(m, k, n_out, xb.esize) if gemm else lib.fcn_inner_product_fwd_workspace_bytes(m, k, n_out, xb.esize))
        ws = DeviceBuffer(nbytes, zero=False) if nbytes else None
        if ws is not None:
            self._keep.append(ws)
        wsp = ws.ptr if ws is not None else None
        flags = (L.CONV_RELU if relu else 0) | (0 if gemm else L.IP_WEIGHTS_NT)
        if xb.esize == 2:
            fn, flags = (lib.fcn_ip_gemm_fwd_f16 if gemm else lib.fcn_inner_product_fwd_f16), flags | (L.CONV_OUT_F32 if yb.esize == 4 else 0)
        else:
            fn = lib.fcn_ip_gemm_fwd_f32 if gemm else lib.fcn_inner_product_fwd_f32
        wptr = devs[0].ptr
        return [Op("ip_gemm" if gemm else "inner_product", l.name, lambda st: L.check(fn(xb.buf.ptr, k, wptr, bias, yb.buf.ptr, yb.cstride, yb.coffset, m, k, n_out,
                                                                  flags, wsp, st)),
                   2.0 * m * c * h * w * n_out, float(xb.esize) * (n_out * k + m * k) + float(yb.esize) * m * n_out)]

    def _fwd_deconvolution(self, l: Layer, halves: List[str]) -> List[Op]:
        lib = L.load()
        g = self._geom(l)
        xb, yb = self.blobs[l.bottoms[0]], self.blobs[l.tops[0]]
        c, co, k = g.cin, g.cout, g.k
        wdev = self.params_dev[l.name][0].ptr
        bdev = self.params_dev[l.name][1].ptr if len(self.params_dev[l.name]) > 1 else None
        if self.param_segs[(l.name, 0)].kind == S.DECONV:
            if self.param_segs[(l.name, 0)].esize == 2:
                return self._fwd_tconv_f16(l, g, xb, yb, wdev, bdev)
            if xb.coffset % 4 or xb.cstride % 4:
                raise NotImplementedError("Deconvolution %s: input view is not 16-byte aligned" % l.name)
            bank = DeviceBuffer(max(int(lib.fcn_tconv_bank_floats(c, co, k, k)), 4) * 4, zero=True)
            d = tconv_desc(xb, yb, g, bank.ptr, bdev)
            tws = DeviceBuffer(int(lib.fcn_tconv2d_workspace_bytes(C.byref(d), 1)), zero=False)
            plan = L.TConvPlan()
            L.call("fcn_tconv2d_prepare", C.byref(d), 1, tws.ptr, -1, C.byref(plan))
            self._keep.extend([bank, d, tws, plan])
            return [Op("tconv_pack", l.name, lambda st: L.check(lib.fcn_tconv_bank_pack_f32(wdev, bank.ptr, c, co, _r4(co), k, k, st)),
                       0.0, 8.0 * c * co * k * k),
                    Op("tconv", l.name, lambda st: L.check(lib.fcn_tconv2d_f32(C.byref(plan), st)),
                       2.0 * g.n * g.h * g.w * c * co * k * k, 4.0 * (xb.pixels * c + yb.pixels * co))]
        if halves and (xb.esize != 2 or xb.coffset % 8):
            raise NotImplementedError("f16 engine: Deconvolution %s from a float32 blob / an unaligned channel slice" % l.name)
        fn, out_f32 = (lib.fcn_deconv_depthwise_fwd_f16, (1 if yb.esize == 4 else 0,)) if halves else (lib.fcn_deconv_depthwise_fwd_f32, ())
        return [Op("deconv", l.name, lambda st: L.check(fn(
            xb.ptr, wdev, bdev, yb.buf.ptr, g.n, g.h, g.w, c, xb.cstride, k, g.s, g.pad, g.oh, g.ow, yb.cstride, yb.coffset, *out_f32, st)),
            2.0 * yb.pixels * c * (k / g.s) ** 2, float(xb.esize * xb.pixels + yb.esize * yb.pixels) * c)]

    def _fwd_tconv_f16(self, l: Layer, g: ConvGeom, xb: Blob, yb: Blob, wdev: int, bdev: Optional[int]) -> List[Op]:
        lib = L.load()
        c, co, k = g.cin, g.cout, g.k
        if xb.esize != 2:
            raise NotImplementedError("f16 engine: Deconvolution %s reads the float32 blob %s" % (l.name, l.bottoms[0]))
        if xb.coffset % 8 or xb.cstride % 8:
            raise NotImplementedError("Deconvolution %s: input view is not 16-byte aligned" % l.name)
        bank = DeviceBuffer(max(int(lib.fcn_tconv_bank_halves(c, co, k, k)), 8) * 2, zero=True)
        d = tconv_desc(xb, yb, g, bank.ptr, bdev, L.CONV_OUT_F32 if yb.esize == 4 else 0)
        tws = DeviceBuffer(int(lib.fcn_tconv2d_workspace_bytes(C.byref(d), 1)), zero=False)
        plan = L.TConvPlan()
        L.call("fcn_tconv2d_prepare_f16", C.byref(d), 1, tws.ptr, -1, C.byref(plan))
        self._keep.extend([bank, d, tws, plan])
        return [Op("tconv_pack", l.name, lambda st: L.check(lib.fcn_tconv_bank_pack_f16(wdev, bank.ptr, c, co, _ra(co, 2), k, k, st)),
                   0.0, 4.0 * c * co * k * k),
                Op("tconv", l.name, lambda st: L.check(lib.fcn_tconv2d_f16(C.byref(plan), st)),
                   2.0 * g.n * g.h * g.w * c * co * k * k, 2.0 * xb.pixels * c + float(yb.esize) * yb.pixels * co)]

    def _stage(self, name: str) -> DeviceBuffer:
        st = self._staging.get(name)
        if st is None:
            b = self.blobs[name]
            st = DeviceBuffer(max(int(np.prod(b.shape)) if b.shape else 1, 1) * 4, zero=False)
            self._staging[name] = st
        return st

    def host_array(self, name: str) -> np.ndarray:
        b = self.blobs[name]
        if b.host is None:
            b.pinned = PinnedArray(b.shape)
            b.host = b.pinned.array
        return b.host

    def _upload_copy(self, name: str, stream: Optional[int]) -> None:
        b = self.blobs[name]
        host = self.host_array(name)
        dst = b.ptr if b.nchw is None else self._stage(name).ptr
        L.check(L.load().fcn_memcpy_h2d_async(dst, host.ctypes.data, host.nbytes, stream))

    def _upload_convert(self, name: str, stream: Optional[int]) -> None:
        b = self.blobs[name]
        if b.nchw is None:
            return
        lib = L.load()
        n, c, h, w = b.nchw
        st = self._stage(name)
        if b.esize == 2:
            L.check(lib.fcn_nchw_f32_to_nhwc_f16(st.ptr, b.buf.ptr, n, c, h, w, b.cstride, b.coffset, b.upload_shift, stream))
        else:
            L.check(lib.fcn_nchw_to_nhwc_f32(st.ptr, b.buf.ptr, n, c, h, w, b.cstride, b.coffset, b.upload_shift, stream))

    def _download_convert(self, name: str, stream: Optional[int]) -> None:
        b = self.blobs[name]
        if b.nchw is None:
            return
        lib = L.load()
        n, c, h, w = b.nchw
        st = self._stage(name)
        if b.esize == 2:
            L.check(lib.fcn_nhwc_f16_to_nchw_f32(b.buf.ptr, st.ptr, n, c, h, w, b.cstride, b.coffset, stream))
        else:
            L.check(lib.fcn_nhwc_to_nchw_f32(b.buf.ptr, st.ptr, n, c, h, w, b.cstride, b.coffset, stream))

    def _download_convert_all(self, stream: Optional[int]) -> None:
        multi = [nm for nm in self.outputs if self.blobs[nm].nchw is not None and self.blobs[nm].esize == 4]
        if 2 <= len(multi) <= 8:
            if not hasattr(self, "_multi_descs"):
                arr = (L.LayoutDesc * len(multi))()
                for d, nm in zip(arr, multi):
                    b = self.blobs[nm]
                    n, c, h, w = b.nchw
                    d.src, d.dst, d.N, d.C, d.H, d.W, d.src_cstride, d.src_coffset = b.buf.ptr, self._stage(nm).ptr, n, c, h, w, b.cstride, b.coffset
                self._multi_descs = arr
            L.check(L.load().fcn_nhwc_to_nchw_multi_f32(self._multi_descs, len(multi), stream))
        else:
            multi = []
        for nm in self.outputs:
            if nm not in multi:
                self._download_convert(nm, stream)

    def _download_copy(self, name: str, stream: Optional[int]) -> None:
        b = self.blobs[name]
        host = self.host_array(name)
        src = b.ptr if b.nchw is None else self._stage(name).ptr
        L.check(L.load().fcn_memcpy_d2h_async(host.ctypes.data, src, host.nbytes, stream))

    def _enqueue_upload(self, name: str, stream: Optional[int]) -> None:
        self._upload_copy(name, stream)
        self._upload_convert(name, stream)

    def _enqueue_download(self, name: str, stream: Optional[int]) -> None:
        self._download_convert(name, stream)
        self._download_copy(name, stream)

    def read_blob(self, name: str) -> np.ndarray:
        if name in self.spec.mask_blobs:
            return self._read_mask(name)
        if name in self.rpn_views:
            return np.ascontiguousarray(self.read_blob(self.rpn_views[name])).reshape(self.shapes[name])
        if name in self.permutes:
            return np.ascontiguousarray(self.read_blob(self.permutes[name]).transpose(0, 2, 3, 1))
        if name in self.spec.prior_blobs:
            return self.prior_consts[name]
        if name in self.detections:
            with self.lock:
                L.call("fcn_init", self.device)
                b = self.blobs[name]
                self.host_array(name)
                if not b.host_valid:
                    self._enqueue_download(name, self.stream)
                    L.call("fcn_stream_sync", self.stream)
                    b.host_valid = True
                return self._compose_detections(name)
        with self.lock:
            L.call("fcn_init", self.device)
            b = self.blobs[name]
            host = self.host_array(name)
            if not b.host_valid:
                for op in self._lazy_blob_ops.get(name, ()):
                    op.run(self.stream)
                self._enqueue_download(name, self.stream)
                L.call("fcn_stream_sync", self.stream)
                if b.lazy_shift:
                    host += F32(b.lazy_shift)
                b.host_valid = True
# ... 7 lines not shown
            host = np.empty((n, c, ph, pw), F32)
            tmp = DeviceBuffer(host.nbytes, zero=False)
            try:
                L.call("fcn_pool_mask_to_nchw_f32", idx.ptr, tmp.ptr, n, ph, pw, c, self.stream)
                L.call("fcn_memcpy_d2h_async", host.ctypes.data, tmp.ptr, host.nbytes, self.stream)
                L.call("fcn_stream_sync", self.stream)
            finally:
                tmp.free()
            return host

    LABEL_TOPS = ("coverage-label", "bbox-label", "size-block", "obj-block", "coverage-block")

    def set_targets(self, rects: Sequence[Sequence[Sequence[int]]], labels: Sequence[Sequence[int]], stride: int,
                    iou_thresh: float = 0.1, tops: Sequence[str] = LABEL_TOPS) -> None:
        fg = self.blobs[tops[0]]
        n, c, gy, gx = fg.shape
        if len(rects) != n or len(labels) != n:
            raise ValueError("need boxes for %d images" % n)
        offs = np.zeros(n + 1, np.int32)
        flat_r, flat_l = [], []
        for i, (rs, ls) in enumerate(zip(rects, labels)):
            for r, lab in zip(rs, ls):
                if not 0 <= int(lab) < c:
                    raise IndexError("label %d outside [0, %d)" % (lab, c))
                flat_r.append([int(v) for v in r])
                flat_l.append(int(lab))
            offs[i + 1] = len(flat_r)
        if not hasattr(self, "_tgt"):
            cap = max(64 * n, 256)
            self._tgt = dict(cap=cap, rects=DeviceBuffer(cap * 16, zero=True), labels=DeviceBuffer(cap * 4, zero=True),
                             offs=DeviceBuffer((n + 1) * 4, zero=True))
        if len(flat_r) > self._tgt["cap"]:
            raise ValueError("too many boxes in one batch (%d > %d)" % (len(flat_r), self._tgt["cap"]))
        self._tgt.update(h_rects=np.asarray(flat_r, np.int32).reshape(-1, 4), h_labels=np.asarray(flat_l, np.int32), h_offs=offs,
                         stride=int(stride), thresh=float(iou_thresh), tops=tuple(tops), pending=True)

    def _enqueue_targets(self) -> None:
        t, lib = self._tgt, L.load()
        if t["h_rects"].size:
            L.check(lib.fcn_memcpy_h2d_async(t["rects"].ptr, t["h_rects"].ctypes.data, t["h_rects"].nbytes, self.stream))
            L.check(lib.fcn_memcpy_h2d_async(t["labels"].ptr, t["h_labels"].ctypes.data, t["h_labels"].nbytes, self.stream))
        L.check(lib.fcn_memcpy_h2d_async(t["offs"].ptr, t["h_offs"].ctypes.data, t["h_offs"].nbytes, self.stream))
        fg, bb, sz, ob, cv = (self.blobs[nm] for nm in t["tops"])
        n, c, gy, gx = fg.shape
        for b in (bb, sz, ob, cv):
            if b.coffset or b.cstride != bb.cstride:
                raise NotImplementedError("label blobs must be plain buffers of one geometry")
        L.check(lib.fcn_gen_targets_nhwc(t["rects"].ptr, t["labels"].ptr, t["offs"].ptr, n, c, gy, gx, t["stride"], t["thresh"],
                                         fg.ptr, fg.cstride, bb.ptr, sz.ptr, ob.ptr, cv.ptr, bb.cstride, self.stream))


    def score_begin(self, io: bool = False) -> None:
        if not self.score_outputs:
            raise RuntimeError("engine was not built with score_outputs=True")
        with self.lock:
            L.call("fcn_init", self.device)
            for nm in self.inputs:
                if nm not in self.device_fed:
                    self.host_array(nm)
                    if self.blobs[nm].nchw is not None:
                        self._stage(nm)
            if graphs_enabled():
                if io and self.graph_io is None:
                    for nm in self.outputs:
                        self.host_array(nm)
                    self.graph_io = self._capture(with_io=True)
                elif not io and self.graph_score is None:
                    self.graph_score = self._capture(with_io=True, download=False)
            for acc in self.score_acc.values():
                L.call("fcn_memset_async", acc.ptr, 0, acc.nbytes, self.stream)
            self.score_forwards = 0

    def forward_score(self, uploaded_event=None) -> None:
        with self.lock:
            for nm in self.inputs:
                if nm not in self.device_fed:
                    self._upload_copy(nm, self.stream)
            if uploaded_event is not None:
                L.call("fcn_event_record", uploaded_event, self.stream)
            if getattr(self, "_tgt", None) is not None and self._tgt.get("pending"):
                self._enqueue_targets()
            if self.graph_score is not None:
                L.call("fcn_graph_launch", self.graph_score, self.stream)
            else:
                for nm in self.inputs:
                    if nm not in self.device_fed:
                        self._upload_convert(nm, self.stream)
                self.run_ops(self.stream)
            for b in self.blobs.values():
                b.host_valid = False
            self.score_forwards += 1

    def score_read(self) -> Dict[str, np.ndarray]:
        with self.lock:
            out = {nm: np.empty(self.blobs[nm].shape, F32) for nm in self.outputs}
            for nm, a in out.items():
                L.call("fcn_memcpy_d2h_async", a.ctypes.data, self.score_acc[nm].ptr, a.nbytes, self.stream)
            L.call("fcn_stream_sync", self.stream)
            return out

    def run_ops(self, stream: Optional[int]) -> None:
        for op in self.ops:
            op.run(stream)

    def _capture(self, with_io: bool, download: bool = True) -> int:
        if with_io:
            for nm in list(self.inputs) + list(self.outputs):
                self.host_array(nm)
                if self.blobs[nm].nchw is not None:
                    self._stage(nm)
        if not getattr(self, "_warm", False):
            self.run_ops(self.stream)
            L.call("fcn_stream_sync", self.stream)
            self._warm = True
        if with_io and not getattr(self, "_warm_io", False):
            for nm in self.inputs:
                if nm not in self.device_fed:
                    self._enqueue_upload(nm, self.stream)
            self._download_convert_all(self.stream)
            for nm in self.outputs:
                self._download_copy(nm, self.stream)
            L.call("fcn_stream_sync", self.stream)
            self._warm_io = True
        L.call("fcn_graph_begin", self.stream)
        try:
            if with_io:
                for nm in self.inputs:
                    if nm not in self.device_fed:
                        self._upload_convert(nm, self.stream)
            self.run_ops(self.stream)
            if with_io and download:
                self._download_convert_all(self.stream)
        finally:
            g = C.c_void_p()
            L.call("fcn_graph_end", self.stream, C.byref(g))
        return int(g.value)

    def _launch_io(self) -> None:
        if self.graph_io is None:
            self.graph_io = self._capture(with_io=True)
        for nm in self.inputs:
            if nm not in self.device_fed:
                self._upload_copy(nm, self.stream)
        L.call("fcn_graph_launch", self.graph_io, self.stream)
        for nm in self.outputs:
            self._download_copy(nm, self.stream)
        self._download_counts(self.stream)

    def forward(self, use_graph: bool = True) -> Dict[str, np.ndarray]:
        use_graph = use_graph and graphs_enabled()
        with self.lock:
            L.call("fcn_init", self.device)
            for nm in self.inputs:
                self.host_array(nm)
            for nm in self.outputs:
                self.host_array(nm)
            if use_graph:
                self._launch_io()
            else:
                for nm in self.inputs:
                    if nm not in self.device_fed:
                        self._enqueue_upload(nm, self.stream)
                self.run_ops(self.stream)
                for nm in self.outputs:
                    self._enqueue_download(nm, self.stream)
                self._download_counts(self.stream)
            L.call("fcn_stream_sync", self.stream)
            for b in self.blobs.values():
                b.host_valid = False
            self._ran = self._counts_valid = True
            out = {}
            for nm in self.outputs:
                b = self.blobs[nm]
                if b.lazy_shift:
                    b.host += F32(b.lazy_shift)
                b.host_valid = True
                out[nm] = self._cut_rois(nm, b.host) if nm not in self.detections else self._compose_detections(nm)
            for nm in self.inputs:
                self.blobs[nm].host_valid = nm not in self.device_fed
            return out

    def forward_begin(self) -> None:
        with self.lock:
            L.call("fcn_init", self.device)
            for nm in list(self.inputs) + list(self.outputs):
                self.host_array(nm)
            if graphs_enabled():
                self._launch_io()
            else:
                for nm in self.inputs:
                    if nm not in self.device_fed:
                        self._enqueue_upload(nm, self.stream)
                self.run_ops(self.stream)
                for nm in self.outputs:
                    self._enqueue_download(nm, self.stream)
                self._download_counts(self.stream)

    def forward_end(self) -> Dict[str, np.ndarray]:
        with self.lock:
            L.call("fcn_stream_sync", self.stream)
            for b in self.blobs.values():
                b.host_valid = False
            self._ran = self._counts_valid = True
            out = {}
            for nm in self.outputs:
                b = self.blobs[nm]
                if b.lazy_shift:
                    b.host += F32(b.lazy_shift)
                b.host_valid = True
                out[nm] = self._cut_rois(nm, b.host) if nm not in self.detections else self._compose_detections(nm)
            for nm in self.inputs:
                self.blobs[nm].host_valid = nm not in self.device_fed
            return out

    def upload_inputs(self) -> None:
        with self.lock:
            for nm in self.inputs:
                self._enqueue_upload(nm, self.stream)
            L.call("fcn_stream_sync", self.stream)

    def forward_enqueue(self) -> None:
        with self.lock:
            if graphs_enabled():
                if self.graph_core is None:
                    self.graph_core = self._capture(with_io=False)
                L.call("fcn_graph_launch", self.graph_core, self.stream)
            else:
                self.run_ops(self.stream)
            for b in self.blobs.values():
                if not b.is_input:
                    b.host_valid = False
            self._ran, self._counts_valid = True, False

    def forward_resident(self, iters: int = 1, use_graph: bool = True) -> float:
        use_graph = use_graph and graphs_enabled()
        with self.lock:
            L.call("fcn_init", self.device)
            if use_graph and self.graph_core is None:
                self.graph_core = self._capture(with_io=False)
            e0, e1 = C.c_void_p(), C.c_void_p()
            L.call("fcn_event_create", C.byref(e0))
            L.call("fcn_event_create", C.byref(e1))
            L.call("fcn_event_record", e0, self.stream)
            for _ in range(iters):
                if use_graph:
                    L.call("fcn_graph_launch", self.graph_core, self.stream)
                else:
                    self.run_ops(self.stream)
            L.call("fcn_event_record", e1, self.stream)
            L.call("fcn_event_sync", e1)
            ms = C.c_float()
            L.call("fcn_event_elapsed_ms", e0, e1, C.byref(ms))
            L.call("fcn_event_destroy", e0)
            L.call("fcn_event_destroy", e1)
            for b in self.blobs.values():
                if not b.is_input:
                    b.host_valid = False
            self._counts_valid = False
            return float(ms.value)

    def time_ops(self, reps: int = 20, ops: Optional[Sequence["Op"]] = None) -> List[Tuple[str, str, float, float, float]]:
        out = []
        with self.lock:
            e0, e1 = C.c_void_p(), C.c_void_p()
            L.call("fcn_event_create", C.byref(e0))
            L.call("fcn_event_create", C.byref(e1))
            for op in (self.ops if ops is None else ops):
                op.run(self.stream)
                L.call("fcn_event_record", e0, self.stream)
                for _ in range(reps):
                    op.run(self.stream)
                L.call("fcn_event_record", e1, self.stream)
                L.call("fcn_event_sync", e1)
                ms = C.c_float()
                L.call("fcn_event_elapsed_ms", e0, e1, C.byref(ms))
                out.append((op.kind, op.name, ms.value / reps, op.flops, op.bytes))
            L.call("fcn_event_destroy", e0)
            L.call("fcn_event_destroy", e1)
        return out

    def time_ops_in_sequence(self, reps: int = 10) -> List[Tuple[str, str, float, float, float]]:
        out = []
        with self.lock:
            e0, e1 = C.c_void_p(), C.c_void_p()
            L.call("fcn_event_create", C.byref(e0))
            L.call("fcn_event_create", C.byref(e1))
            ms = C.c_float()
            empty = []
            for _ in range(10):
                self.ops[0].run(self.stream)
                L.call("fcn_event_record", e0, self.stream)
                L.call("fcn_event_record", e1, self.stream)
                L.call("fcn_event_sync", e1)
                L.call("fcn_event_elapsed_ms", e0, e1, C.byref(ms))
                empty.append(ms.value)
            floor = float(np.median(empty))
            for i, op in enumerate(self.ops):
                acc = []
                for _ in range(reps):
                    for prev in self.ops[:i]:
                        prev.run(self.stream)
                    L.call("fcn_event_record", e0, self.stream)
                    op.run(self.stream)
                    L.call("fcn_event_record", e1, self.stream)
                    L.call("fcn_event_sync", e1)
                    L.call("fcn_event_elapsed_ms", e0, e1, C.byref(ms))
                    acc.append(ms.value)
                out.append((op.kind, op.name, float(np.median(acc)), op.flops, op.bytes))
            L.call("fcn_event_destroy", e0)
            L.call("fcn_event_destroy", e1)
        self.event_pair_floor_ms = floor
        return out

    def close(self) -> None:
        with self.lock:
            lib = L.load()
            for g in (self.graph_io, self.graph_core, self.graph_score):
                if g:
                    lib.fcn_graph_destroy(g)
            self.graph_io = self.graph_core = self.graph_score = None
# ... 22 lines not shown
                 max_lds_kb: Optional[int] = 36, **engine_kw):
        if depth < 1:
            raise ValueError("depth must be at least 1")
        self.engines: List[Engine] = []
        if os.environ.get("FCN_PIPE_LDS_KB"):
            max_lds_kb = int(os.environ["FCN_PIPE_LDS_KB"]) or None
        if max_lds_kb is not None:
            engine_kw.setdefault("tune_max_lds_kb", max_lds_kb)
        for i in range(depth):
            self.engines.append(Engine(make_spec(), params=params, device=device, tune_from=self.engines[0] if i else None, replica=i,
                                       **engine_kw))
        self._pending: List[Engine] = []
        self._next = 0

    @property
    def depth(self) -> int:
        return len(self.engines)

    def submit(self, inputs: Dict[str, np.ndarray]) -> None:
        if len(self._pending) >= len(self.engines):
            raise RuntimeError("ForwardPipeline: %d frames already in flight, collect() one first" % len(self._pending))
        eng = self.engines[self._next]
        self._next = (self._next + 1) % len(self.engines)
        for nm, arr in inputs.items():
            eng.host_array(nm)[...] = arr
        eng.forward_begin()
        self._pending.append(eng)

    def collect(self) -> Dict[str, np.ndarray]:
        if not self._pending:
            raise RuntimeError("ForwardPipeline: nothing in flight")
        eng = self._pending.pop(0)
        return {k: v.copy() for k, v in eng.forward_end().items()}

    def map(self, frames: Sequence[Dict[str, np.ndarray]]) -> List[Dict[str, np.ndarray]]:
        out: List[Dict[str, np.ndarray]] = []
        for f in frames:
            if len(self._pending) == len(self.engines):
                out.append(self.collect())
            self.submit(f)
        while self._pending:
            out.append(self.collect())
        return out

    def calibrate(self, depths: Sequence[int] = (3, 4), iters: int = 60) -> int:
        best, best_t = None, 1e30
        for d in depths:
            if 1 <= d <= len(self.engines):
                self.run_resident(iters, depth=d)
                t = self.run_resident(iters, depth=d)
                if t < best_t:
                    best, best_t = d, t
        self.active = best or len(self.engines)
        return self.active

    def run_resident(self, iters: int, depth: Optional[int] = None) -> float:
        import time
        lib = L.load()
        engines = self.engines[:depth or getattr(self, "active", None) or len(self.engines)]
        return self._run_resident(engines, iters, lib, time)

    def run_io(self, iters: int, depth: Optional[int] = None) -> float:
        import time
        engines = self.engines[:depth or getattr(self, "active", None) or len(self.engines)]
        pending: List[Engine] = []
        t0 = time.perf_counter()
        for i in range(iters):
            e = engines[i % len(engines)]
            if len(pending) == len(engines):
                pending.pop(0).forward_end()
            e.forward_begin()
            pending.append(e)
        while pending:
            pending.pop(0).forward_end()
        return time.perf_counter() - t0

    def warm_io(self, depth: Optional[int] = None) -> None:
        for e in self.engines[:depth or getattr(self, "active", None) or len(self.engines)]:
            e.forward_begin()
            e.forward_end()

    def _run_resident(self, engines, iters, lib, time) -> float:
        for e in engines:
            if e.graph_core is None:
                e.forward_resident(1)
            L.call("fcn_stream_sync", e.stream)
        no_graph = not graphs_enabled()
        t0 = time.perf_counter()
        for i in range(iters):
            e = engines[i % len(engines)]
            if no_graph:
                e.run_ops(e.stream)
            else:
                L.check(lib.fcn_graph_launch(e.graph_core, e.stream))
        for e in engines:
            L.call("fcn_stream_sync", e.stream)
        return time.perf_counter() - t0

    def close(self) -> None:
        for e in self.engines:
            e.close()
```

fcn_object_detector_amd/lib.py:

```python
from __future__ import annotations

import ctypes as C
import os
import threading
from typing import Optional

_HERE = os.path.dirname(os.path.abspath(__file__))
LIB_PATH = os.environ.get("FCN_LIB_PATH") or os.path.join(_HERE, "libfcnhip.so")


class FcnLibraryError(RuntimeError):
    pass


class FcnError(RuntimeError):
    def __init__(self, code: int, msg: str):
        super().__init__("libfcnhip error %d: %s" % (code, msg))
        self.code = code


class ConvDesc(C.Structure):
    _fields_ = [
        ("x", C.c_void_p), ("w", C.c_void_p), ("bias", C.c_void_p), ("y", C.c_void_p), ("y2", C.c_void_p),
        ("N", C.c_int32), ("H", C.c_int32), ("W", C.c_int32), ("Cin", C.c_int32), ("x_cstride", C.c_int32),
# ... 121 lines not shown
    _fields_ = [(k, C.c_int32) for k in ("H", "W", "A", "feat_stride", "pre_nms_topn", "post_nms_topn")] + [
        ("min_size", C.c_float), ("nms_thresh", C.c_float)] + [(k, C.c_int32) for k in (
            "score_cstride", "score_coffset", "delta_cstride", "delta_coffset", "rois_cstride", "rois_coffset", "top_score_cstride",
            "top_score_coffset")] + [("anchors", C.c_float * 128)]


PROPOSAL_MAX_ANCHORS = 32
PROPOSAL_MAX_CANDIDATES = 65536
PROPOSAL_MAX_PRE_NMS = 6144
SSD_MAX_HEADS = 16
DETOUT_MAX_TOPK = 1024
CODE_CORNER, CODE_CENTER_SIZE = 1, 2
CONV_RELU, CONV_SIGMOID2, CONV_ACCUM, CONV_OUT_F32, CONV_F16, CONV_OUT_F16, CONV_MASK = 1, 2, 4, 8, 16, 32, 64
IP_MAX_ROWS = 32
IP_WEIGHTS_NT = 256


def ip_rows_refusal(layer: str, rows: int) -> str:
    return ("InnerProduct %s: a batch of %d rows (the streaming kernels take at most %d): the matrix-core kernels take any row count for "
            "a NetSpec built with ip_gemm=True (caffe.Net, the solvers and the caffe tool pass it)" % (layer, rows, IP_MAX_ROWS))
CONV_IMAGE_ONES = 128
ELT_PROD, ELT_SUM, ELT_MAX = 0, 1, 2
ARGMAX_MAX_TOPK = 32
ACT_PRELU, ACT_TANH, ACT_BIAS = 0, 1, 2
ACT_MODES = {"PReLU": ACT_PRELU, "TanH": ACT_TANH, "Bias": ACT_BIAS}
ARGMAX_WAVE_BYTES, ARGMAX_WAVE_PIXELS, ARGMAX_WAVE_MIN_C = 512, 8192, 32
ARGMAX_VALUES, ARGMAX_PAIRS, ARGMAX_SOFTMAX = 1, 2, 4
SOLVER_KINDS = {"SGD": 0, "NESTEROV": 1, "ADAGRAD": 2, "RMSPROP": 3, "ADADELTA": 4, "ADAM": 5}
REG_L2, REG_L1 = 0, 1
RECT_ROUND_NEAREST_EVEN, RECT_ROUND_TRUNCATE = 0, 1

_vp, _i, _f, _d, _sz = C.c_void_p, C.c_int, C.c_float, C.c_double, C.c_size_t

PROTOTYPES = {
    "fcn_abi_version": (_i, []),
    "fcn_last_error_string": (C.c_char_p, []),
    "fcn_device_count": (_i, [C.POINTER(_i)]),
    "fcn_init": (_i, [_i]),
    "fcn_device_name": (_i, [C.c_char_p, _i]),
    "fcn_device_sync": (_i, []),
    "fcn_malloc": (_i, [C.POINTER(_vp), _sz]),
    "fcn_free": (_i, [_vp]),
    "fcn_host_malloc": (_i, [C.POINTER(_vp), _sz]),
    "fcn_host_free": (_i, [_vp]),
    "fcn_memset_async": (_i, [_vp, _i, _sz, _vp]),
    "fcn_memcpy_h2d_async": (_i, [_vp, _vp, _sz, _vp]),
    "fcn_memcpy_d2h_async": (_i, [_vp, _vp, _sz, _vp]),
    "fcn_memcpy_d2d_async": (_i, [_vp, _vp, _sz, _vp]),
    "fcn_stream_create": (_i, [C.POINTER(_vp)]),
    "fcn_stream_destroy": (_i, [_vp]),
    "fcn_stream_sync": (_i, [_vp]),
    "fcn_event_create": (_i, [C.POINTER(_vp)]),
    "fcn_event_destroy": (_i, [_vp]),
    "fcn_event_record": (_i, [_vp, _vp]),
    "fcn_event_sync": (_i, [_vp]),
    "fcn_event_elapsed_ms": (_i, [_vp, _vp, C.POINTER(_f)]),
    "fcn_graph_begin": (_i, [_vp]),
    "fcn_graph_end": (_i, [_vp, C.POINTER(_vp)]),
    "fcn_graph_launch": (_i, [_vp, _vp]),
    "fcn_graph_destroy": (_i, [_vp]),
    "fcn_stream_create_replica": (_i, [C.POINTER(_vp), _i]),
    "fcn_stream_is_prioritized": (_i, [_vp, C.POINTER(_i)]),
    "fcn_nchw_to_nhwc_f32": (_i, [_vp, _vp, _i, _i, _i, _i, _i, _i, _f, _vp]),
    "fcn_nhwc_to_nchw_f32": (_i, [_vp, _vp, _i, _i, _i, _i, _i, _i, _vp]),
    "fcn_nhwc_to_nchw_multi_f32": (_i, [C.POINTER(LayoutDesc), _i, _vp]),
    "fcn_conv2d_fwd_f32": (_i, [C.POINTER(ConvDesc), _vp]),
    "fcn_conv2d_group_workspace_bytes": (_sz, [_i]),
    "fcn_conv2d_num_configs": (_i, []),
    "fcn_conv2d_first_layer_config": (_i, []),
    "fcn_conv2d_config_lds_bytes": (_i, [_i]),
    "fcn_conv2d_config_waves_k": (_i, [_i]),
    "fcn_conv2d_group_prepare": (_i, [C.POINTER(ConvDesc), _i, _vp, _i, C.POINTER(ConvGroup)]),
    "fcn_conv2d_group_prepare_fused": (_i, [C.POINTER(ConvDesc), _i, C.POINTER(PoolDesc), _i, _vp, _i, C.POINTER(ConvGroup)]),
    "fcn_conv2d_fwd_group_f32": (_i, [C.POINTER(ConvGroup), _vp]),
    "fcn_conv2d_group_release": (_i, [_vp]),
    "fcn_conv2d_tail_scratch_bytes": (C.c_size_t, [C.POINTER(ConvTail)]),
    "fcn_conv2d_tail_arrive_bytes": (C.c_size_t, [C.POINTER(ConvTail)]),
    "fcn_conv2d_group_attach_tail": (_i, [_vp, C.POINTER(ConvTail)]),
    "fcn_maxpool_fwd_f32": (_i, [_vp, _vp, _vp] + [_i] * 12 + [_vp]),
    "fcn_avepool_fwd_f32": (_i, [_vp, _vp] + [_i] * 12 + [_vp]),
    "fcn_lrn_fwd_f32": (_i, [_vp, _vp, _vp, _i, _i, _i, _i, _i, _f, _f, _f, _vp]),
    "fcn_maxpool_lrn5_fwd_f32": (_i, [_vp, _vp] + [_i] * 12 + [_f, _f, _f, _vp]),
    "fcn_maxpool_lrn5_fwd_f16": (_i, [_vp, _vp] + [_i] * 12 + [_f, _f, _f, _vp]),
    "fcn_maxpool_lrn5_conv1x1_fwd_f32": (_i, [_vp] + [_i] * 10 + [_f, _f, _f, _vp, _vp, _i, _i, _vp, _i, _i, _vp]),
    "fcn_maxpool_lrn5_conv1x1_fwd_f16": (_i, [_vp] + [_i] * 10 + [_f, _f, _f, _vp, _vp, _i, _i, _vp, _i, _i, _vp]),
    "fcn_relu_fwd_f32": (_i, [_vp, _vp, _sz, _f, _vp]),
    "fcn_sigmoid_fwd_f32": (_i, [_vp, _vp, _sz, _vp]),
    "fcn_power_fwd_f32": (_i, [_vp, _vp, _sz, _f, _f, _f, _vp]),
    "fcn_eltwise_fwd_f32": (_i, [_vp, _vp, _vp, _sz, _i, _f, _f, _vp]),
    "fcn_copy_channels_f32": (_i, [_vp, _vp, _i, _i, _i, _i, _i, _i, _vp]),
    "fcn_deconv_depthwise_fwd_f32": (_i, [_vp, _vp, _vp, _vp] + [_i] * 12 + [_vp]),
    "fcn_preprocess_bgr8": (_i, [_vp, _i, _i, _vp, _i, _i, _i, _f, _vp, _vp]),
    "fcn_detect_workspace_bytes": (_sz, [C.POINTER(DetectParams), _i]),
    "fcn_detect_decode_group": (_i, [_vp, _vp, _i, _sz, _sz, C.POINTER(DetectParams), _vp, _vp, _vp, _vp, _vp]),
    "fcn_score_masks_workspace_bytes": (_sz, [_i, _i, _i, _i]),
    "fcn_score_masks": (_i, [_vp, _i, _i, _i, _i, _i, _i, _vp, _f, _vp, _i, _i, _vp, _vp, _vp]),
    "fcn_gen_targets": (_i, [_vp, _vp, _vp, _i, _i, _i, _i, _i, _d, _vp, _vp, _vp, _vp, _vp, _vp]),
    "fcn_gen_targets_nhwc": (_i, [_vp, _vp, _vp, _i, _i, _i, _i, _i, _d, _vp, _i, _vp, _vp, _vp, _vp, _i, _vp]),
    "fcn_conv2d_wgrad_workspace_floats": (_sz, [C.POINTER(ConvDesc), C.POINTER(_i)]),
    "fcn_conv2d_wgrad_f32": (_i, [C.POINTER(ConvDesc), _vp, _vp, _vp, _vp]),
    "fcn_conv2d_wgrad_group_workspace_floats": (_sz, [C.POINTER(ConvDesc), _i]),
    "fcn_conv2d_wgrad_group_f32": (_i, [C.POINTER(ConvDesc), _vp, _vp, _i, _vp, _vp]),
    "fcn_conv2d_wgrad_num_configs": (_i, []),
    "fcn_conv2d_wgrad_split_config": (_i, []),
    "fcn_conv2d_wgrad_workspace_floats_cfg": (_sz, [C.POINTER(ConvDesc), _i, C.POINTER(_i)]),
    "fcn_conv2d_wgrad_cfg_f32": (_i, [C.POINTER(ConvDesc), _vp, _vp, _vp, _i, _vp]),
    "fcn_conv2d_wgrad_group_workspace_floats_cfg": (_sz, [C.POINTER(ConvDesc), _i, _i]),
    "fcn_conv2d_wgrad_group_cfg_f32": (_i, [C.POINTER(ConvDesc), _vp, _vp, _i, _vp, _i, _vp]),
    "fcn_conv_weights_flip_f32": (_i, [_vp, _vp, _i, _i, _i, _i, _i, _i, _vp]),
    "fcn_nchw_f32_to_nhwc_f16": (_i, [_vp, _vp, _i, _i, _i, _i, _i, _i, _f, _vp]),
    "fcn_nhwc_f16_to_nchw_f32": (_i, [_vp, _vp, _i, _i, _i, _i, _i, _i, _vp]),
    "fcn_maxpool_fwd_f16": (_i, [_vp, _vp] + [_i] * 12 + [_vp]),
    "fcn_lrn_fwd_f16": (_i, [_vp, _vp, _i, _i, _i, _i, _i, _f, _f, _f, _vp]),
    "fcn_avepool_fwd_f16": (_i, [_vp, _vp] + [_i] * 12 + [_vp]),
    "fcn_deconv_depthwise_fwd_f16": (_i, [_vp, _vp, _vp, _vp] + [_i] * 13 + [_vp]),
    "fcn_eltwise_fwd_f16": (_i, [_vp, _vp, _vp, _sz, _i, _f, _f, _vp]),
    "fcn_softmax_fwd_f16": (_i, [_vp, _vp, _i, _i, _i, _i, _i, _vp]),
    "fcn_copy_channels_f16": (_i, [_vp, _vp, _i, _i, _i, _i, _i, _i, _vp]),
    "fcn_preprocess_bgr8_batch": (_i, [_vp, _i, _i, _i, _vp, _i, _i, _i, _i, _f, _vp, _vp]),
    "fcn_preprocess_bgr8_rois": (_i, [_vp, _i, _i, _vp, _i, _vp, _i, _i, _i, _i, _f, _vp, _vp]),
    "fcn_preprocess_bgr8_f16": (_i, [_vp, _i, _i, _vp, _i, _i, _i, _f, _vp, _vp]),
    "fcn_compose_scene_bgr8": (_i, [_vp, _i, _i, _i, _i, _i, _i, _vp, _i, _i, _vp, _vp, _i, _i, _vp]),
    "fcn_mask_to_label_f32": (_i, [_vp, _i, _i, _vp, _i, _i, _i, _vp]),
    "fcn_compose_scene_view_bgr8": (_i, [_vp, _i, _i, _i, _i, _i, _i, _vp, _i, _i, _vp, _vp, _i, _i, _i, _i, _i, _i, _vp]),
    "fcn_blur_gauss_bgr8": (_i, [_vp, _vp, _vp, _i, _i, _vp, _i, _vp]),
    "fcn_blur_box_bgr8": (_i, [_vp, _vp, _i, _i, _i, _vp]),
    "fcn_blur_median_bgr8": (_i, [_vp, _vp, _i, _i, _i, _vp]),
    "fcn_color_augment_bgr8": (_i, [_vp, _vp, _i, _i, _vp, _vp]),
    "fcn_softmax_fwd_f32": (_i, [_vp, _vp, _i, _i, _i, _i, _vp]),
    "fcn_softmax_loss_workspace_bytes": (_sz, []),
    "fcn_softmax_loss_f32": (_i, [_vp, _vp, _vp, _vp, _i, _i, _i, _i, _i, _i, _i, _i, _f, _vp, _vp]),
    "fcn_deconv_depthwise_bwd_f32": (_i, [_vp, _vp, _vp] + [_i] * 13 + [_vp]),
    "fcn_conv_weights_flip_batch_f32": (_i, [_vp, _vp, _vp, _i, _vp]),
    "fcn_relu_bwd_f32": (_i, [_vp, _vp, _vp, _i, _i, _i, _vp]),
    "fcn_relu_bwd_slope_f32": (_i, [_vp, _vp, _vp, _i, _i, _i, _f, _i, _vp]),
    "fcn_sigmoid_bwd_f32": (_i, [_vp, _vp, _vp, _sz, _i, _vp]),
    "fcn_maxpool_bwd_f32": (_i, [_vp, _vp, _vp] + [_i] * 14 + [_vp]),
    "fcn_maxpool_bwd_mask_f32": (_i, [_vp, _vp, _vp] + [_i] * 14 + [_vp, _i, _i, _vp]),
    "fcn_avepool_bwd_f32": (_i, [_vp, _vp] + [_i] * 14 + [_vp]),
    "fcn_lrn_bwd_f32": (_i, [_vp, _vp, _vp, _vp, _vp, _i, _i, _i, _i, _i, _f, _f, _i, _vp]),
    "fcn_dropout_f32": (_i, [_vp, _vp] + [_i] * 8 + [_f, C.c_uint, C.c_uint, _vp]),
    "fcn_stream_wait_event": (_i, [_vp, _vp]),
    "fcn_comm_unique_id": (_i, [C.c_char_p]),
    "fcn_comm_init": (_i, [C.POINTER(_vp), C.c_char_p, _i, _i]),
    "fcn_comm_allreduce_sum_f32": (_i, [_vp, _vp, _sz, _vp]),
    "fcn_comm_destroy": (_i, [_vp]),
    "fcn_loss_f32": (_i, [_i, _vp, _vp, _vp, _vp, _i, _i, _i, _i, _f, _vp]),
    "fcn_sgd_update_f32": (_i, [_vp, _vp, _vp, _vp, _i, _f, _f, _f, _f, _vp]),
    "fcn_adam_update_f32": (_i, [_vp, _vp, _vp, _vp, _vp, _i, _f, _f, _f, _f, _f, _i, _f, _vp]),
    "fcn_solver_update_f32": (_i, [_i, _vp, _vp, _vp, _vp, _vp, _i, _f, _f, _f, _f, _f, _f, _i, _i, _f, _vp, _vp]),
    "fcn_grad_clip_workspace_bytes": (_sz, []),
    "fcn_grad_clip_f32": (_i, [_vp, _vp, _i, _f, _f, _vp, _vp, _vp, _vp]),
    "fcn_grad_accumulate_f32": (_i, [_vp, _vp, _sz, _i, _vp]),
    "fcn_score_accumulate_f32": (_i, [_vp, _vp, _i, _i, _i, _i, _i, _vp]),
    "fcn_accuracy_workspace_bytes": (_sz, []),
    "fcn_accuracy_f32": (_i, [_vp, _vp, _vp, _vp, _i, _i, _i, _i, _i, _i, _i, _i, _vp, _vp]),
    "fcn_tconv2d_num_configs": (_i, []),
    "fcn_tconv2d_workspace_bytes": (_sz, [C.POINTER(TConvDesc), _i]),
    "fcn_tconv2d_prepare": (_i, [C.POINTER(TConvDesc), _i, _vp, _i, C.POINTER(TConvPlan)]),
    "fcn_tconv2d_f32": (_i, [C.POINTER(TConvPlan), _vp]),
    "fcn_tconv_bank_floats": (_sz, [_i, _i, _i, _i]),
    "fcn_tconv_bank_pack_f32": (_i, [_vp, _vp, _i, _i, _i, _i, _i, _vp]),
    "fcn_tconv2d_num_configs_f16": (_i, []),
    "fcn_tconv2d_prepare_f16": (_i, [C.POINTER(TConvDesc), _i, _vp, _i, C.POINTER(TConvPlan)]),
    "fcn_tconv2d_f16": (_i, [C.POINTER(TConvPlan), _vp]),
    "fcn_tconv_bank_halves": (_sz, [_i, _i, _i, _i]),
# ... 132 lines not shown
```

fcn_object_detector_amd/tune.py:

```python
from __future__ import annotations

import ctypes as C
import json
import os
from typing import Callable, Dict, Iterable, List, NamedTuple, Optional, Sequence, Tuple

import numpy as np

from . import engine as E
from . import lib as L


def lower_quartile(samples: Sequence[float]) -> float:
    return float(np.percentile(samples, 25))


class Protocol(NamedTuple):
    warm: int
    reps: int
    evict: bool
    samples: int
    stat: Callable[[Sequence[float]], float]
    contenders: int
    margin: float
# ... 71 lines not shown
        L.call("fcn_event_record", e1, self.stream)
        L.call("fcn_event_sync", e1)
        ms = C.c_float()
        L.call("fcn_event_elapsed_ms", e0, e1, C.byref(ms))
        return ms.value / reps

    def fastest(self, cfgs: Iterable[int], prepare: Callable[[int], bool], launch: Callable[[], None], p: Protocol,
                second_look: bool = True) -> Tuple[int, float]:
        timed: List[Tuple[float, int]] = []
        for cfg in cfgs:
            if not prepare(cfg):
                continue
            for _ in range(p.warm):
                launch()
            timed.append((p.stat([self.measure(launch, p.reps, p.evict) for _ in range(p.samples)]), cfg))
        if not timed:
            return -1, 1e30
        best_ms, best = min(timed)
        if second_look and len(timed) > 1:
            finals = []
            for t1, cfg in sorted(timed)[:p.contenders]:
                if t1 > p.margin * best_ms:
                    break
                if prepare(cfg):
                    finals.append((p.stat(([t1] if p.carry else []) + [self.measure(launch, p.reps, p.evict) for _ in range(p.look)]), cfg))
            if finals:
                best_ms, best = min(finals)
        return best, best_ms

    def time_conv_cfgs(self, arr, n: int, ws: "E.DeviceBuffer", parr=None, npool: int = 0) -> Tuple[int, float]:
        lib = L.load()
        grp = L.ConvGroup()
        first_layer = int(lib.fcn_conv2d_first_layer_config())
        cold = self.cold and os.environ.get("FCN_TUNE_COLD", "1") != "0"

        def admitted(cfg: int) -> bool:
            if cfg == first_layer:
                return os.environ.get("FCN_CONV_FIRST7", "1") != "0"
            return int(lib.fcn_conv2d_config_lds_bytes(cfg)) <= self.max_lds

        def prepare(cfg: int) -> bool:
            return lib.fcn_conv2d_group_prepare_fused(arr, n, parr, npool, ws.ptr, cfg, C.byref(grp)) == 0

        return self.fastest([c for c in range(int(lib.fcn_conv2d_num_configs())) if admitted(c)], prepare,
                            lambda: L.check(lib.fcn_conv2d_fwd_group_f32(C.byref(grp), self.stream)), COLD if cold else WARM,
                            cold or os.environ.get("FCN_TUNE_SECOND_LOOK", "1") != "0")

    def _subset_ms(self, descs: Sequence[L.ConvDesc], pools: Sequence[L.PoolDesc] = ()) -> float:
        lib = L.load()
        arr = (L.ConvDesc * len(descs))(*descs)
        parr = (L.PoolDesc * max(len(pools), 1))(*pools) if pools else None
        ws = E.DeviceBuffer(int(lib.fcn_conv2d_group_workspace_bytes(len(descs))), zero=False)
        try:
            return self.time_conv_cfgs(arr, len(descs), ws, parr, len(pools))[1]
        finally:
            L.call("fcn_conv2d_group_release", ws.ptr)
            ws.free()

    def choose(self, key: str, valid: Callable[[object], bool], search: Callable[[], object]):
        for known in (self.tune_from, self.cache):
            if known is not None and valid(known.get(key)):
                value = known[key]
                break
        else:
            value = search()
            if self.cache is not None:
                self.cache[key] = value
                try:
                    with open(self.cache_path, "w") as f:
                        json.dump(self.cache, f, indent=0, sort_keys=True)
                except OSError:
                    pass
        self.chosen[key] = value
        return value

    @staticmethod
    def _valid_cfg(ncfg: int) -> Callable[[object], bool]:
        return lambda v: type(v) is int and 0 <= v < ncfg

    def conv_cfg(self, name: str, arr, n: int, ws: "E.DeviceBuffer", parr=None, npool: int = 0) -> int:
        return self.choose(self.key(name), self._valid_cfg(int(L.load().fcn_conv2d_num_configs())),
                           lambda: self.time_conv_cfgs(arr, n, ws, parr, npool)[0])

    def wgrad_cfgs(self, ops: Sequence["E.Op"]) -> None:
        ncfg = int(L.load().fcn_conv2d_wgrad_num_configs())
        for op in ops:
            if op.kind != "wgrad" or op.sel is None:
                continue

            def select(cfg: int) -> bool:
                op.sel["cfg"] = cfg
                return True

            op.sel["cfg"] = self.choose(self.key("wgrad:" + "+".join(op.layers)), self._valid_cfg(ncfg),
                                        lambda: self.fastest(range(ncfg), select, lambda: op.run(self.stream), WGRAD)[0])
            op.name += " [cfg%d]" % op.sel["cfg"]

    def split_level(self, chunk: List["E.ConvTask"]) -> List[List["E.ConvTask"]]:
        n = len(chunk)
        if n < 2 or n > 4:
            return [chunk]

        def valid(code) -> bool:
            return isinstance(code, str) and len(code) == n and all(ch.isdigit() and int(ch) < n for ch in code)

        def search() -> str:
            memo: Dict[Tuple[int, ...], float] = {}

            def cost(sub: Tuple[int, ...]) -> float:
                if sub not in memo:
                    memo[sub] = self._subset_ms([chunk[i].desc for i in sub])
                return memo[sub]

            best, best_ms = None, 1e30
            for labels in set_partitions(n):
                ms = sum(cost(tuple(i for i in range(n) if labels[i] == g)) for g in sorted(set(labels)))
                if ms < best_ms - 1e-7:
                    best, best_ms = labels, ms
            return "".join(str(g) for g in best)

        choice = self.choose("cut|" + self.key("+".join(it.layer.name for it in chunk)), valid, search)
        groups: Dict[str, List[E.ConvTask]] = {}
        for it, g in zip(chunk, choice):
            groups.setdefault(g, []).append(it)
        return [groups[g] for g in sorted(groups)]

    def move_floaters(self, tasks: Sequence[object], levels: List[int]) -> None:
        for lv in range(max(levels, default=-1)):
            a_idx, b_idx = ([i for i, t in enumerate(tasks) if levels[i] == l2 and isinstance(t, E.ConvTask)] for l2 in (lv, lv + 1))
            if len(a_idx) < 2 or not b_idx or len(a_idx) > 8:
                continue
            fl = [i for i in a_idx if E.task_floats(tasks, levels, i)]
            if not fl or len(fl) > 3 or len(b_idx) + len(fl) > 8:
                continue

            def valid(code) -> bool:
                return isinstance(code, str) and len(code) == len(fl) and set(code) <= {"0", "1"} and (len(fl) < len(a_idx) or "0" in code)

            def search() -> str:
                pools = {l2: [t.pool_desc for j, t in enumerate(tasks) if levels[j] == l2 and isinstance(t, E.OpTask) and t.pool_desc is not None][:2]
                         for l2 in (lv, lv + 1)}
                memo: Dict[Tuple[int, Tuple[int, ...]], float] = {}

                def cost(l2: int, sub: Tuple[int, ...]) -> float:
                    if (l2, sub) not in memo:
                        memo[(l2, sub)] = min(self._subset_ms([tasks[i].desc for i in sub], pools[l2]) for _ in range(2))
                    return memo[(l2, sub)]

                best, best_ms, base_ms = "0" * len(fl), None, None
                for code in range(1 << len(fl)):
                    moved = [fl[b] for b in range(len(fl)) if code >> b & 1]
                    stay = tuple(i for i in a_idx if i not in moved)
                    if not stay:
                        continue
                    ms = cost(lv, stay) + cost(lv + 1, tuple(b_idx + moved))
                    if code == 0:
                        base_ms = ms
                    if best_ms is None or ms < best_ms:
                        best, best_ms = "".join("1" if code >> b & 1 else "0" for b in range(len(fl))), ms
                if best_ms > float(os.environ.get("FCN_MOVE_MARGIN", "0.99")) * base_ms:
                    best = "0" * len(fl)
                return best

            names = ("+".join(tasks[i].layer.name for i in idx) for idx in (a_idx, b_idx))
            choice = self.choose("move|" + self.key(">".join(names)), valid, search)
            for b, i in enumerate(fl):
# ... 3 lines not shown
```

include/fcnhip.h:

```cpp
#ifndef FCNHIP_H_
#define FCNHIP_H_

#include <stddef.h>
#include <stdint.h>

#ifdef __cplusplus
extern "C" {
#endif

#define FCN_ABI_VERSION 2

#define FCN_E_ARG       1
#define FCN_E_ALIGN     2
#define FCN_E_UNSUPPORTED 3
#define FCN_E_STATE     4
#define FCN_E_CAPACITY  5

typedef void* fcn_stream_t;
typedef void* fcn_event_t;
typedef void* fcn_graph_t;
typedef void* fcn_comm_t;

int  fcn_abi_version(void);
const char* fcn_last_error_string(void);
// ... 26 lines not shown
int  fcn_stream_create_replica(fcn_stream_t* s, int index);
int  fcn_stream_is_prioritized(fcn_stream_t s, int* h_yes);

int  fcn_nchw_to_nhwc_f32(const float* src, float* dst, int N, int C, int H, int W,
                          int dst_cstride, int dst_coffset, float shift, fcn_stream_t s);
int  fcn_nhwc_to_nchw_f32(const float* src, float* dst, int N, int C, int H, int W,
                          int src_cstride, int src_coffset, fcn_stream_t s);
typedef struct fcn_layout_desc {
    const float* src;
    float* dst;
    int32_t N, C, H, W, src_cstride, src_coffset;
} fcn_layout_desc;
int  fcn_nhwc_to_nchw_multi_f32(const fcn_layout_desc* h_descs, int n, fcn_stream_t s);

#define FCN_CONV_RELU      1
#define FCN_CONV_SIGMOID2  2
#define FCN_CONV_ACCUM     4
#define FCN_CONV_MASK     64
#define FCN_CONV_IMAGE_ONES 128
#define FCN_CONV_OUT_F32   8
#define FCN_CONV_OUT_F16  32
#define FCN_CONV_F16      16
typedef struct fcn_conv_desc {
    const float* x;
    const float* w;
    const float* bias;
    float*       y;
    float*       y2;
    int32_t N, H, W, Cin, x_cstride;
    int32_t Cout, kh, kw, pad, stride, OH, OW;
    int32_t y_cstride, y_coffset, y2_cstride, y2_coffset;
    int32_t flags;
    float   in_shift;
} fcn_conv_desc;
int  fcn_conv2d_fwd_f32(const fcn_conv_desc* h_desc, fcn_stream_t s);
typedef struct fcn_conv_group {
    void*   d_probs;
    int32_t n;
    int32_t cfg;
    int32_t total_tiles;
} fcn_conv_group;
size_t fcn_conv2d_group_workspace_bytes(int n);
int  fcn_conv2d_num_configs(void);
int  fcn_conv2d_first_layer_config(void);
typedef struct fcn_conv_tail {
    int32_t n;
    int32_t finalize;
    fcn_conv_desc heads[4];
    float*  scratch;
    void*   arrive;
} fcn_conv_tail;
size_t fcn_conv2d_tail_scratch_bytes(const fcn_conv_tail* t);
size_t fcn_conv2d_tail_arrive_bytes(const fcn_conv_tail* t);
int  fcn_conv2d_group_attach_tail(void* d_workspace, const fcn_conv_tail* t);
int  fcn_conv2d_config_lds_bytes(int cfg);
int  fcn_conv2d_config_waves_k(int cfg);
int  fcn_conv2d_group_prepare(const fcn_conv_desc* h_descs, int n, void* d_workspace, int cfg_request, fcn_conv_group* h_out);
int  fcn_conv2d_fwd_group_f32(const fcn_conv_group* h_group, fcn_stream_t s);
typedef struct fcn_pool_desc {
    const float* x; float* y; int32_t* idx;
    int32_t N, H, W, C, x_cstride, k, stride, pad, OH, OW, y_cstride, y_coffset;
    int32_t f16;
} fcn_pool_desc;
int  fcn_conv2d_group_prepare_fused(const fcn_conv_desc* h_descs, int n, const fcn_pool_desc* h_pools, int npools, void* d_workspace,
                                    int cfg_request, fcn_conv_group* h_out);
int  fcn_conv2d_group_release(void* d_workspace);

int  fcn_maxpool_fwd_f32(const float* x, float* y, int32_t* idx, int N, int H, int W, int C,
                         int x_cstride, int k, int stride, int pad, int OH, int OW,
                         int y_cstride, int y_coffset, fcn_stream_t s);
int  fcn_avepool_fwd_f32(const float* x, float* y, int N, int H, int W, int C, int x_cstride,
                         int k, int stride, int pad, int OH, int OW, int y_cstride, int y_coffset,
                         fcn_stream_t s);
int  fcn_lrn_fwd_f32(const float* x, float* y, float* scale, int pixels, int C, int x_cstride,
                     int y_cstride, int local_size, float alpha, float beta, float k, fcn_stream_t s);
int  fcn_maxpool_lrn5_fwd_f32(const float* x, float* y, int N, int H, int W, int C, int x_cstride, int k, int stride, int pad,
                              int OH, int OW, int y_cstride, int lrn_first, float alpha, float beta, float lrn_k, fcn_stream_t s);
int  fcn_maxpool_lrn5_conv1x1_fwd_f32(const float* x, int N, int H, int W, int C, int x_cstride, int k, int stride, int pad,
                                      int OH, int OW, float alpha, float beta, float lrn_k, const float* w, const float* bias,
                                      int Cout, int relu, float* y, int y_cstride, int y_coffset, fcn_stream_t s);
int  fcn_maxpool_lrn5_conv1x1_fwd_f16(const void* x, int N, int H, int W, int C, int x_cstride, int k, int stride, int pad,
                                      int OH, int OW, float alpha, float beta, float lrn_k, const void* w, const float* bias,
                                      int Cout, int relu, void* y, int y_cstride, int y_coffset, fcn_stream_t s);
int  fcn_relu_fwd_f32(const float* x, float* y, size_t count, float negative_slope, fcn_stream_t s);
int  fcn_sigmoid_fwd_f32(const float* x, float* y, size_t count, fcn_stream_t s);
int  fcn_power_fwd_f32(const float* x, float* y, size_t count, float power, float scale, float shift, fcn_stream_t s);
#define FCN_ELT_PROD 0
#define FCN_ELT_SUM  1
#define FCN_ELT_MAX  2
int  fcn_eltwise_fwd_f32(const float* a, const float* b, float* y, size_t count, int op,
                         float ca, float cb, fcn_stream_t s);
int  fcn_copy_channels_f32(const float* src, float* dst, int pixels, int C, int src_cstride,
                           int src_coffset, int dst_cstride, int dst_coffset, fcn_stream_t s);
int  fcn_softmax_fwd_f32(const float* x, float* y, int pixels, int C, int x_cstride, int y_cstride, fcn_stream_t s);
int  fcn_deconv_depthwise_fwd_f32(const float* x, const float* w, const float* bias, float* y,
                                  int N, int H, int W, int C, int x_cstride, int k, int stride, int pad,
                                  int OH, int OW, int y_cstride, int y_coffset, fcn_stream_t s);

int  fcn_preprocess_bgr8(const uint8_t* frame, int h, int w, float* dst, int H, int W, int dst_cstride,
                         float shift, float* d_minmax, fcn_stream_t s);

int  fcn_nchw_f32_to_nhwc_f16(const float* src, void* dst, int N, int C, int H, int W, int dst_cstride, int dst_coffset, float shift,
                              fcn_stream_t s);
int  fcn_nhwc_f16_to_nchw_f32(const void* src, float* dst, int N, int C, int H, int W, int src_cstride, int src_coffset, fcn_stream_t s);
int  fcn_maxpool_fwd_f16(const void* x, void* y, int N, int H, int W, int C, int x_cstride, int k, int stride, int pad, int OH, int OW,
                         int y_cstride, int y_coffset, fcn_stream_t s);
int  fcn_lrn_fwd_f16(const void* x, void* y, int pixels, int C, int x_cstride, int y_cstride, int local_size, float alpha, float beta,
                     float k, fcn_stream_t s);
int  fcn_maxpool_lrn5_fwd_f16(const void* x, void* y, int N, int H, int W, int C, int x_cstride, int k, int stride, int pad,
                              int OH, int OW, int y_cstride, int lrn_first, float alpha, float beta, float lrn_k, fcn_stream_t s);
int  fcn_avepool_fwd_f16(const void* x, void* y, int N, int H, int W, int C, int x_cstride, int k, int stride, int pad, int OH, int OW,
                         int y_cstride, int y_coffset, fcn_stream_t s);
int  fcn_deconv_depthwise_fwd_f16(const void* x, const float* w, const float* bias, void* y, int N, int H, int W, int C, int x_cstride,
                                  int k, int stride, int pad, int OH, int OW, int y_cstride, int y_coffset, int out_f32, fcn_stream_t s);
int  fcn_eltwise_fwd_f16(const void* a, const void* b, void* y, size_t count, int op, float ca, float cb, fcn_stream_t s);
int  fcn_softmax_fwd_f16(const void* x, void* y, int pixels, int C, int x_cstride, int y_cstride, int out_f32, fcn_stream_t s);
int  fcn_copy_channels_f16(const void* src, void* dst, int pixels, int C, int src_cstride, int src_coffset, int dst_cstride,
                           int dst_coffset, fcn_stream_t s);
int  fcn_preprocess_bgr8_rois(const uint8_t* frame, int h, int w, const int32_t* h_rois, int n, void* dst, int dst_f16, int H, int W,
                              int dst_cstride, float shift, float* d_minmax, fcn_stream_t s);
int  fcn_preprocess_bgr8_batch(const uint8_t* frames, int n, int h, int w, void* dst, int dst_f16, int H, int W, int dst_cstride,
                               float shift, float* d_minmax, fcn_stream_t s);
int  fcn_preprocess_bgr8_f16(const uint8_t* frame, int h, int w, void* dst, int H, int W, int dst_cstride, float shift, float* d_minmax,
                             fcn_stream_t s);

typedef struct fcn_scene_obj {
    const uint8_t* img;
    const uint8_t* mask;
    int32_t src_h, src_w;
    int32_t flip;
    int32_t roi_x, roi_y, roi_w, roi_h;
    int32_t out_w, out_h;
    int32_t cx, cy;
    int32_t label1;
} fcn_scene_obj;
int  fcn_compose_scene_bgr8(const uint8_t* bg, int bg_h, int bg_w, int crop_x, int crop_y, int crop_w, int crop_h,
                            const fcn_scene_obj* d_objs, int nobj, int final_flip, uint8_t* out_img, uint8_t* out_mask,
                            int H, int W, fcn_stream_t s);
int  fcn_compose_scene_view_bgr8(const uint8_t* bg, int bg_h, int bg_w, int crop_x, int crop_y, int crop_w, int crop_h,
                                 const fcn_scene_obj* d_objs, int nobj, int final_flip, uint8_t* out_img, uint8_t* out_mask,
                                 int H, int W, int view_x, int view_y, int view_w, int view_h, fcn_stream_t s);

#define FCN_GAUSS_MAX_RADIUS 15
int  fcn_blur_gauss_bgr8(const uint8_t* src, uint8_t* dst, float* tmp, int h, int w, const float* h_taps, int radius, fcn_stream_t s);
int  fcn_blur_box_bgr8(const uint8_t* src, uint8_t* dst, int h, int w, int k, fcn_stream_t s);
int  fcn_blur_median_bgr8(const uint8_t* src, uint8_t* dst, int h, int w, int k, fcn_stream_t s);
typedef struct fcn_color_params {
    float sharpen_centre;
    float sharpen_off;
    int32_t add[3];
    float mul[3];
    float gray_alpha;
    float gray_keep;
} fcn_color_params;
int  fcn_color_augment_bgr8(const uint8_t* src, uint8_t* dst, int h, int w, const fcn_color_params* h_params, fcn_stream_t s);

int  fcn_mask_to_label_f32(const uint8_t* mask, int h, int w, float* dst, int H, int W, int dst_cstride, fcn_stream_t s);

#define FCN_RECT_ROUND_NEAREST_EVEN 0
#define FCN_RECT_ROUND_TRUNCATE     1
typedef struct fcn_detect_params {
    int32_t num_classes;
    int32_t gy, gx;
    int32_t cell_w, cell_h;
    int32_t cvg_cstride, cvg_coffset;
    int32_t box_cstride, box_coffset;
// ... 339 lines not shown
```

Baseline: 4514 frames/s.

## Fuse 7x7 stem conv, maxpool, LRN and 1x1 conv into one kernel

Adds a stem kernel that computes the first 7x7 stride-2 convolution with MFMA into LDS, then applies maxpool, LRN and the following 1x1 convolution within the same workgroup. It can read the planar NCHW input directly, skipping the separate layout conversion. The goal is to avoid writing and re-reading the large first-layer activation and to drop several kernel launches. The cost is extra halo recompute, since spare waves compute an additional row, and added LDS pressure. An autotuner picks between the split and fused forms, and lazy input staging adds host-side state complexity.

```diff
diff --git a/fcn_object_detector_amd/csrc/conv_fwd.hip b/fcn_object_detector_amd/csrc/conv_fwd.hip
--- a/fcn_object_detector_amd/csrc/conv_fwd.hip
+++ b/fcn_object_detector_amd/csrc/conv_fwd.hip
@@ -6,6 +6,7 @@
 
 #include "common.h"
 #include "conv_common.h"
+#include "first7_loop.h"
 
 using namespace fcn;
 
@@ -989,13 +990,10 @@
     conv_body<T, WTM, WTN, WAVES_M, WAVES_N, WAVES_K, BK, NBUF, PF>(p, blockIdx.x, smem);
 }
 
-constexpr int kD7Th = 8, kD7Tw = 32;
-constexpr int kD7Ph = 2 * kD7Th + 5, kD7Pw = 2 * kD7Tw + 6;
-constexpr int kD7RowF = kD7Pw * 3;
+constexpr int kD7Th = 8;
+constexpr int kD7Ph = 2 * kD7Th + 5;
 constexpr int kD7PatchF = kD7Ph * kD7RowF;
-constexpr int kD7WRowF = 22, kD7WPitchF = 7 * kD7WRowF;
 constexpr int kD7WOff = (kD7PatchF + 3) / 4 * 4;
-constexpr int kD7EpiPitch = 68;
 constexpr int kD7StageF = kD7WOff + 64 * kD7WPitchF;
 constexpr int kD7EpiF = 4 * 2 * 32 * kD7EpiPitch;
 constexpr int kD7LdsBytes = (kD7StageF > kD7EpiF ? kD7StageF : kD7EpiF) * 4;
@@ -1066,26 +1064,7 @@
             for (int e = 0; e < 16; ++e) acc[i][j][e] = 0.f;
     __syncthreads();
     FCN_STAMP(2);
-    auto frag = [&](const int step, float (&a)[2], float (&b)[2]) {
-        const int r = step / 11, j = step - 11 * r;
-#pragma unroll
-        for (int mt = 0; mt < 2; ++mt) a[mt] = a_base[(2 * mt + r) * kD7RowF + 2 * j];
-#pragma unroll
-        for (int nt = 0; nt < 2; ++nt) b[nt] = b_base[nt * 32 * kD7WPitchF + r * kD7WRowF + 2 * j];
-    };
-    float fa[3][2], fb[3][2];
-    frag(0, fa[0], fb[0]);
-    frag(1, fa[1], fb[1]);
-#pragma unroll
-    for (int step = 0; step < 77; ++step) {
-        if (step + 2 < 77) frag(step + 2, fa[(step + 2) % 3], fb[(step + 2) % 3]);
-        __builtin_amdgcn_sched_barrier(0);
-#pragma unroll
-        for (int mt = 0; mt < 2; ++mt)
-#pragma unroll
-            for (int nt = 0; nt < 2; ++nt)
-                acc[mt][nt] = __builtin_amdgcn_mfma_f32_32x32x2f32(fa[step % 3][mt], fb[step % 3][nt], acc[mt][nt], 0, 0, 0);
-    }
+    FCN_FIRST7_MFMA_LOOP(a_base, b_base, acc, false, a_base, b_base, acc[0][0]);
     FCN_STAMP(3);
     __syncthreads();
     float* epi = smem + wave * (2 * 32 * kD7EpiPitch);
diff --git a/fcn_object_detector_amd/csrc/first7_loop.h b/fcn_object_detector_amd/csrc/first7_loop.h
--- /dev/null
+++ b/fcn_object_detector_amd/csrc/first7_loop.h
@@ -0,0 +1,48 @@
+#pragma once
+
+#include "conv_common.h"
+
+namespace fcn {
+
+constexpr int kD7Tw = 32;
+constexpr int kD7Pw = 2 * kD7Tw + 6;
+constexpr int kD7RowF = kD7Pw * 3;
+constexpr int kD7WRowF = 22, kD7WPitchF = 7 * kD7WRowF;
+constexpr int kD7EpiPitch = 68;
+
+}
+
+#define FCN_FIRST7_MFMA_LOOP(a_base, b_base, acc, XT, xa, xb, xacc)                                                                       \
+        auto frag = [&](const int step, float (&a)[2], float (&b)[2]) {                                              \
+            const int r = step / 11, j = step - 11 * r;                                                                                   \
+            _Pragma("unroll") for (int mt = 0; mt < 2; ++mt) a[mt] = (a_base)[(2 * mt + r) * kD7RowF + 2 * j];                            \
+            _Pragma("unroll") for (int nt = 0; nt < 2; ++nt) b[nt] = (b_base)[nt * 32 * kD7WPitchF + r * kD7WRowF + 2 * j];               \
+        };                                                                                                                                \
+                                           \
+        float fa[3][2], fb[3][2];                                                                                                         \
+        [[maybe_unused]] float fx[3][2];                                                                                                  \
+        [[maybe_unused]] auto fragx = [&](const int step, float (&x)[2]) {                                                                \
+            if constexpr (XT) {                                                                                                           \
+                const int r = step / 11, j = step - 11 * r;                                                                               \
+                x[0] = (xa)[r * kD7RowF + 2 * j];                                                                                         \
+                x[1] = (xb)[r * kD7WRowF + 2 * j];                                                                                        \
+            }                                                                                                                             \
+        };                                                                                                                                \
+        frag(0, fa[0], fb[0]);                                                                                                            \
+        frag(1, fa[1], fb[1]);                                                                                                            \
+        if constexpr (XT) {                                                                                                               \
+            fragx(0, fx[0]);                                                                                                              \
+            fragx(1, fx[1]);                                                                                                              \
+        }                                                                                                                                 \
+        _Pragma("unroll") for (int step = 0; step < 77; ++step) {                                                                         \
+            if (step + 2 < 77) {                                                                                                          \
+                frag(step + 2, fa[(step + 2) % 3], fb[(step + 2) % 3]);                                                                   \
+                if constexpr (XT) fragx(step + 2, fx[(step + 2) % 3]);                                                                    \
+            }                                                                                                                             \
+                                                        \
+            __builtin_amdgcn_sched_barrier(0);                                                                                            \
+            _Pragma("unroll") for (int mt = 0; mt < 2; ++mt)                                                                              \
+                _Pragma("unroll") for (int nt = 0; nt < 2; ++nt)                                                                          \
+                    (acc)[mt][nt] = __builtin_amdgcn_mfma_f32_32x32x2f32(fa[step % 3][mt], fb[step % 3][nt], (acc)[mt][nt], 0, 0, 0);     \
+            if constexpr (XT) (xacc) = __builtin_amdgcn_mfma_f32_32x32x2f32(fx[step % 3][0], fx[step % 3][1], (xacc), 0, 0, 0);           \
+        }
diff --git a/fcn_object_detector_amd/csrc/lrn_common.h b/fcn_object_detector_amd/csrc/lrn_common.h
--- /dev/null
+++ b/fcn_object_detector_amd/csrc/lrn_common.h
@@ -0,0 +1,46 @@
+#pragma once
+
+#include "common.h"
+
+namespace fcn {
+
+__device__ __forceinline__ float4 ld4(const float* p) { return *reinterpret_cast<const float4*>(p); }
+__device__ __forceinline__ void st4(float* p, float4 v) { *reinterpret_cast<float4*>(p) = v; }
+
+__device__ __forceinline__ float pow_neg_beta(float s, float beta) {
+    if (beta == 0.75f) {
+        const float r = sqrtf(s);
+        return 1.f / (r * sqrtf(r));
+    }
+    return powf(s, -beta);
+}
+
+__device__ __forceinline__ float pow_neg_beta_fast(float s, float beta) {
+    if (beta == 0.75f) {
+        const float r = __builtin_amdgcn_rsqf(s);
+        return r * __builtin_amdgcn_sqrtf(r);
+    }
+    return powf(s, -beta);
+}
+
+template <bool FAST = false>
+__device__ __forceinline__ float4 lrn5_apply(const float4 l, const float4 c, const float4 r, float alpha_over_n, float beta, float kk, float4& s) {
+    const float q[12] = {l.x * l.x, l.y * l.y, l.z * l.z, l.w * l.w, c.x * c.x, c.y * c.y,
+                         c.z * c.z, c.w * c.w, r.x * r.x, r.y * r.y, r.z * r.z, r.w * r.w};
+    s.x = kk + alpha_over_n * (q[2] + q[3] + q[4] + q[5] + q[6]);
+    s.y = kk + alpha_over_n * (q[3] + q[4] + q[5] + q[6] + q[7]);
+    s.z = kk + alpha_over_n * (q[4] + q[5] + q[6] + q[7] + q[8]);
+    s.w = kk + alpha_over_n * (q[5] + q[6] + q[7] + q[8] + q[9]);
+    float4 o;
+    o.x = c.x * (FAST ? pow_neg_beta_fast(s.x, beta) : pow_neg_beta(s.x, beta));
+    o.y = c.y * (FAST ? pow_neg_beta_fast(s.y, beta) : pow_neg_beta(s.y, beta));
+    o.z = c.z * (FAST ? pow_neg_beta_fast(s.z, beta) : pow_neg_beta(s.z, beta));
+    o.w = c.w * (FAST ? pow_neg_beta_fast(s.w, beta) : pow_neg_beta(s.w, beta));
+    return o;
+}
+
+__device__ __forceinline__ float4 max4(const float4 a, const float4 b) {
+    return make_float4(b.x > a.x ? b.x : a.x, b.y > a.y ? b.y : a.y, b.z > a.z ? b.z : a.z, b.w > a.w ? b.w : a.w);
+}
+
+}
diff --git a/fcn_object_detector_amd/csrc/pointwise.hip b/fcn_object_detector_amd/csrc/pointwise.hip
--- a/fcn_object_detector_amd/csrc/pointwise.hip
+++ b/fcn_object_detector_amd/csrc/pointwise.hip
@@ -2,13 +2,11 @@
 #include <math.h>
 
 #include "common.h"
+#include "lrn_common.h"
 
 using namespace fcn;
 
 namespace {
-
-__device__ __forceinline__ float4 ld4(const float* p) { return *reinterpret_cast<const float4*>(p); }
-__device__ __forceinline__ void st4(float* p, float4 v) { *reinterpret_cast<float4*>(p) = v; }
 
 template <typename D>
 __global__ __launch_bounds__(256) void nchw_to_nhwc_kernel(const float* __restrict__ src, D* __restrict__ dst,
@@ -180,38 +178,6 @@
     }
 }
 
-__device__ __forceinline__ float pow_neg_beta(float s, float beta) {
-    if (beta == 0.75f) {
-        const float r = sqrtf(s);
-        return 1.f / (r * sqrtf(r));
-    }
-    return powf(s, -beta);
-}
-
-__device__ __forceinline__ float pow_neg_beta_fast(float s, float beta) {
-    if (beta == 0.75f) {
-        const float r = __builtin_amdgcn_rsqf(s);
-        return r * __builtin_amdgcn_sqrtf(r);
-    }
-    return powf(s, -beta);
-}
-
-template <bool FAST = false>
-__device__ __forceinline__ float4 lrn5_apply(const float4 l, const float4 c, const float4 r, float alpha_over_n, float beta, float kk, float4& s) {
-    const float q[12] = {l.x * l.x, l.y * l.y, l.z * l.z, l.w * l.w, c.x * c.x, c.y * c.y,
-                         c.z * c.z, c.w * c.w, r.x * r.x, r.y * r.y, r.z * r.z, r.w * r.w};
-    s.x = kk + alpha_over_n * (q[2] + q[3] + q[4] + q[5] + q[6]);
-    s.y = kk + alpha_over_n * (q[3] + q[4] + q[5] + q[6] + q[7]);
-    s.z = kk + alpha_over_n * (q[4] + q[5] + q[6] + q[7] + q[8]);
-    s.w = kk + alpha_over_n * (q[5] + q[6] + q[7] + q[8] + q[9]);
-    float4 o;
-    o.x = c.x * (FAST ? pow_neg_beta_fast(s.x, beta) : pow_neg_beta(s.x, beta));
-    o.y = c.y * (FAST ? pow_neg_beta_fast(s.y, beta) : pow_neg_beta(s.y, beta));
-    o.z = c.z * (FAST ? pow_neg_beta_fast(s.z, beta) : pow_neg_beta(s.z, beta));
-    o.w = c.w * (FAST ? pow_neg_beta_fast(s.w, beta) : pow_neg_beta(s.w, beta));
-    return o;
-}
-
 __global__ __launch_bounds__(256) void lrn5_kernel(const float* __restrict__ x, float* __restrict__ y, float* __restrict__ scale,
                                                    long long pixels, int C, int x_cstride, int y_cstride, float alpha_over_n,
                                                    float beta, float kk) {
@@ -229,10 +195,6 @@
         st4(y + (size_t)pix * y_cstride + g * 4, o);
         if (scale) st4(scale + (size_t)pix * C + g * 4, s);
     }
-}
-
-__device__ __forceinline__ float4 max4(const float4 a, const float4 b) {
-    return make_float4(b.x > a.x ? b.x : a.x, b.y > a.y ? b.y : a.y, b.z > a.z ? b.z : a.z, b.w > a.w ? b.w : a.w);
 }
 
 template <bool LRN_FIRST>
diff --git a/fcn_object_detector_amd/csrc/stem.hip b/fcn_object_detector_amd/csrc/stem.hip
--- /dev/null
+++ b/fcn_object_detector_amd/csrc/stem.hip
@@ -0,0 +1,238 @@
+#include <float.h>
+#include <math.h>
+
+#include "common.h"
+#include "conv_common.h"
+#include "first7_loop.h"
+#include "lrn_common.h"
+
+using namespace fcn;
+
+namespace {
+
+constexpr int kStRows = 9, kStPoolH = 4, kStPoolW = 15;
+constexpr int kStPh = 2 * kStRows + 5;
+constexpr int kStPatchF = kStPh * kD7RowF;
+constexpr int kStWOff = (kStPatchF + 3) / 4 * 4;
+constexpr int kStStageF = kStWOff + 64 * kD7WPitchF;
+constexpr int kStImgF = kStRows * 32 * kD7EpiPitch;
+constexpr int kStActPitch = 68, kStActF = 64 * kStActPitch;
+constexpr int kStLdsBytes = (kStStageF > kStImgF ? kStStageF : kStImgF) * 4;
+constexpr int kStThreads = 256;
+static_assert(kStLdsBytes <= 80 * 1024, "stem kernel: tile workgroups of other frames must fit beside it");
+static_assert(kStActF <= kStImgF && kStPoolH * kStPoolW <= 64 && 2 * (kStPoolH - 1) + 2 < kStRows && 2 * (kStPoolW - 1) + 2 < 32 - 1, "stem patch");
+
+struct StemP {
+    const float* x;
+    const float* w1;
+    const float* b1;
+    const float* w2;
+    const float* b2;
+    float* y;
+    int H, W, CH, CW, OH, OW, patches_x, patches_y;
+    int y_cstride, y_coffset, relu1, relu2;
+    float shift, alpha_over_n, beta, kk;
+};
+
+template <bool PLANAR>
+__global__ __launch_bounds__(kStThreads) void stem_fwd_kernel(const StemP p) {
+#if defined(__HIP_DEVICE_COMPILE__)
+    __shared__ __attribute__((aligned(16))) float smem[kStLdsBytes / 4];
+    const int tid = threadIdx.x, lane = tid & 63, wave = __builtin_amdgcn_readfirstlane(tid >> 6);
+    int t = blockIdx.x;
+    const int Q = t % p.patches_x;
+    t /= p.patches_x;
+    const int P = t % p.patches_y, n = t / p.patches_y;
+    const int cy0 = 2 * kStPoolH * P, cx0 = 2 * kStPoolW * Q;
+    const int iy0 = 2 * cy0 - 3, ix0 = 2 * cx0 - 3;
+    const v4f zero4 = {0.f, 0.f, 0.f, 0.f};
+    constexpr int PI = (kStPh * kD7Pw + kStThreads - 1) / kStThreads, WI = (64 * 49 + kStThreads - 1) / kStThreads;
+    v4f px[PI], wv[WI];
+    const size_t plane = (size_t)p.H * p.W;
+    const float* xn = p.x + (size_t)n * plane * (PLANAR ? 3 : 4);
+#pragma unroll
+    for (int i = 0; i < PI; ++i) {
+        const int s = tid + kStThreads * i;
+        const int pr = s / kD7Pw, pc = s - pr * kD7Pw;
+        const int iy = iy0 + pr, ix = ix0 + pc;
+        const bool ok = s < kStPh * kD7Pw && (unsigned)iy < (unsigned)p.H && (unsigned)ix < (unsigned)p.W;
+        if constexpr (PLANAR) {
+            const float* xp = xn + (size_t)(ok ? iy : 0) * p.W + (ok ? ix : 0);
+            px[i][0] = ok ? xp[0] + p.shift : 0.f;
+            px[i][1] = ok ? xp[plane] + p.shift : 0.f;
+            px[i][2] = ok ? xp[2 * plane] + p.shift : 0.f;
+            px[i][3] = 0.f;
+        } else {
+            px[i] = ok ? *reinterpret_cast<const v4f*>(xn + ((size_t)iy * p.W + ix) * 4) : zero4;
+        }
+    }
+#pragma unroll
+    for (int i = 0; i < WI; ++i) {
+        const int tp = tid + kStThreads * i;
+        wv[i] = tp < 64 * 49 ? *reinterpret_cast<const v4f*>(p.w1 + (size_t)tp * 4) : zero4;
+    }
+#pragma unroll
+    for (int i = 0; i < PI; ++i) {
+        const int s = tid + kStThreads * i;
+        if (s < kStPh * kD7Pw) {
+            float* d = smem + s * 3;
+            d[0] = px[i][0]; d[1] = px[i][1]; d[2] = px[i][2];
+        }
+    }
+#pragma unroll
+    for (int i = 0; i < WI; ++i) {
+        const int tp = tid + kStThreads * i;
+        if (tp < 64 * 49) {
+            const int co = tp / 49, rq = tp - co * 49;
+            const int r = rq / 7, q = rq - r * 7;
+            float* d = smem + kStWOff + co * kD7WPitchF + r * kD7WRowF + q * 3;
+            d[0] = wv[i][0]; d[1] = wv[i][1]; d[2] = wv[i][2];
+        }
+    }
+    for (int i = tid; i < 64 * 7; i += kStThreads) smem[kStWOff + i * kD7WRowF + 21] = 0.f;
+    const int nl = lane & 31, h = lane >> 5;
+    const float bias_lo = p.b1 ? p.b1[nl] : 0.f, bias_hi = p.b1 ? p.b1[nl + 32] : 0.f;
+    const float* a_base = smem + (4 * wave) * kD7RowF + 6 * nl + h;
+    const float* b_base = smem + kStWOff + nl * kD7WPitchF + h;
+    const float* ax_base = smem + 2 * (kStRows - 1) * kD7RowF + 6 * nl + h;
+    const float* bx_base = b_base + (wave & 1) * 32 * kD7WPitchF;
+    f32x16 acc[2][2], accx;
+#pragma unroll
+    for (int e = 0; e < 16; ++e) {
+        accx[e] = 0.f;
+#pragma unroll
+        for (int i = 0; i < 2; ++i)
+#pragma unroll
+            for (int j = 0; j < 2; ++j) acc[i][j][e] = 0.f;
+    }
+    __syncthreads();
+    if (wave < 2) {
+        FCN_FIRST7_MFMA_LOOP(a_base, b_base, acc, true, ax_base, bx_base, accx);
+    } else {
+        FCN_FIRST7_MFMA_LOOP(a_base, b_base, acc, false, ax_base, bx_base, accx);
+    }
+    const int fi = lane & 15, fh = lane >> 4;
+    const float* wp = p.w2 + (size_t)(16 * wave + fi) * 64 + 16 * fh;
+    float4 wf[4];
+#pragma unroll
+    for (int j = 0; j < 4; ++j) wf[j] = ld4(wp + 4 * j);
+    const float4 bv = p.b2 ? ld4(p.b2 + 16 * wave + 4 * fh) : make_float4(0.f, 0.f, 0.f, 0.f);
+    __syncthreads();
+    const bool relu1 = p.relu1 != 0;
+    auto put = [&](const f32x16& a, const int row, const int nt) {
+        const float b = nt ? bias_hi : bias_lo;
+        float* d = smem + (row * 32 + 4 * h) * kD7EpiPitch + nl + 32 * nt;
+#pragma unroll
+        for (int v = 0; v < 16; ++v) {
+            float o = a[v] + b;
+            if (relu1) o = fmaxf(o, 0.f);
+            d[((v & 3) + 8 * (v >> 2)) * kD7EpiPitch] = o;
+        }
+    };
+#pragma unroll
+    for (int mt = 0; mt < 2; ++mt)
+#pragma unroll
+        for (int nt = 0; nt < 2; ++nt) put(acc[mt][nt], 2 * wave + mt, nt);
+    if (wave < 2) put(accx, kStRows - 1, wave);
+    __syncthreads();
+    float4 a0[2], a1[2];
+#pragma unroll
+    for (int pass = 0; pass < 2; ++pass) {
+        const int item = tid + kStThreads * pass;
+        const int pp = min(item >> 3, kStPoolH * kStPoolW - 1), q = item & 7;
+        const int ly = pp / kStPoolW, lx = pp - kStPoolW * ly;
+        const int oy = min(kStPoolH * P + ly, p.OH - 1), ox = min(kStPoolW * Q + lx, p.OW - 1);
+        const int hs = 2 * oy, ws = 2 * ox;
+        const int h1 = min(hs + 3, p.CH) - 1, w1 = min(ws + 3, p.CW) - 1;
+        const float* ib = smem + 8 * q;
+        float4 t0[9], t1[9];
+#pragma unroll
+        for (int r = 0; r < 3; ++r)
+#pragma unroll
+            for (int c = 0; c < 3; ++c) {
+                const int iy = min(hs + r, h1) - cy0, ix = min(ws + c, w1) - cx0;
+                const float* ip = ib + (iy * 32 + ix) * kD7EpiPitch;
+                t0[3 * r + c] = ld4(ip);
+                t1[3 * r + c] = ld4(ip + 4);
+            }
+        float4 m0 = t0[0], m1 = t1[0];
+#pragma unroll
+        for (int i = 1; i < 9; ++i) {
+            m0 = max4(m0, t0[i]);
+            m1 = max4(m1, t1[i]);
+        }
+        float4 lft, rgt;
+        lft.x = __shfl_up(m1.x, 1); lft.y = __shfl_up(m1.y, 1); lft.z = __shfl_up(m1.z, 1); lft.w = __shfl_up(m1.w, 1);
+        rgt.x = __shfl_down(m0.x, 1); rgt.y = __shfl_down(m0.y, 1); rgt.z = __shfl_down(m0.z, 1); rgt.w = __shfl_down(m0.w, 1);
+        const float4 zero = make_float4(0.f, 0.f, 0.f, 0.f);
+        if (q == 0) lft = zero;
+        if (q == 7) rgt = zero;
+        float4 s;
+        a0[pass] = lrn5_apply<true>(lft, m0, m1, p.alpha_over_n, p.beta, p.kk, s);
+        a1[pass] = lrn5_apply<true>(m0, m1, rgt, p.alpha_over_n, p.beta, p.kk, s);
+    }
+    __syncthreads();
+#pragma unroll
+    for (int pass = 0; pass < 2; ++pass) {
+        const int item = tid + kStThreads * pass;
+        st4(smem + (item >> 3) * kStActPitch + 8 * (item & 7), a0[pass]);
+        st4(smem + (item >> 3) * kStActPitch + 8 * (item & 7) + 4, a1[pass]);
+    }
+    __syncthreads();
+#pragma unroll
+    for (int tt = 0; tt < 4; ++tt) {
+        const float* ap = smem + (16 * tt + fi) * kStActPitch + 16 * fh;
+        float4 af[4];
+#pragma unroll
+        for (int j = 0; j < 4; ++j) af[j] = ld4(ap + 4 * j);
+        v4f o4 = {0.f, 0.f, 0.f, 0.f};
+#pragma unroll
+        for (int j = 0; j < 4; ++j) {
+            o4 = __builtin_amdgcn_mfma_f32_16x16x4f32(wf[j].x, af[j].x, o4, 0, 0, 0);
+            o4 = __builtin_amdgcn_mfma_f32_16x16x4f32(wf[j].y, af[j].y, o4, 0, 0, 0);
+            o4 = __builtin_amdgcn_mfma_f32_16x16x4f32(wf[j].z, af[j].z, o4, 0, 0, 0);
+            o4 = __builtin_amdgcn_mfma_f32_16x16x4f32(wf[j].w, af[j].w, o4, 0, 0, 0);
+        }
+        float4 o = make_float4(o4[0] + bv.x, o4[1] + bv.y, o4[2] + bv.z, o4[3] + bv.w);
+        if (p.relu2) o = make_float4(fmaxf(o.x, 0.f), fmaxf(o.y, 0.f), fmaxf(o.z, 0.f), fmaxf(o.w, 0.f));
+        const int pp = 16 * tt + fi;
+        const int ly = pp / kStPoolW, lx = pp - kStPoolW * ly;
+        const int py = kStPoolH * P + ly, pxx = kStPoolW * Q + lx;
+        if (pp < kStPoolH * kStPoolW && py < p.OH && pxx < p.OW)
+            st4(p.y + ((size_t)(n * p.OH + py) * p.OW + pxx) * p.y_cstride + p.y_coffset + 16 * wave + 4 * fh, o);
+    }
+#endif
+}
+
+inline bool aligned16(const void* q) { return ((uintptr_t)q & 15) == 0; }
+
+}
+
+extern "C" {
+
+int fcn_stem_fwd_f32(const float* x, int planar, float shift, int N, int H, int W, const float* w1, const float* b1, int relu1, float alpha,
+                     float beta, float lrn_k, const float* w2, const float* b2, int relu2, float* y, int OH, int OW, int y_cstride, int y_coffset,
+                     fcn_stream_t s) {
+    FCN_REQUIRE(x && w1 && w2 && y && N > 0 && H > 0 && W > 0 && OH > 0 && OW > 0 && y_coffset >= 0, FCN_E_ARG, "stem: bad args");
+    FCN_REQUIRE(y_cstride >= y_coffset + 64, FCN_E_ARG, "stem: channel stride smaller than the channels");
+    const int CH = (H - 1) / 2 + 1, CW = (W - 1) / 2 + 1;
+    FCN_REQUIRE((OH - 1) * 2 < CH && (OW - 1) * 2 < CW, FCN_E_ARG, "stem: OH x OW = %d x %d too large for the %d x %d pixels of conv1", OH, OW, CH, CW);
+    FCN_REQUIRE(aligned16(w1) && aligned16(w2) && (!b2 || aligned16(b2)) && aligned16(y) && y_cstride % 4 == 0 && y_coffset % 4 == 0 &&
+                (planar || aligned16(x)), FCN_E_UNSUPPORTED, "stem: needs 16-byte channel groups");
+    const long long px = cdiv(OW, kStPoolW), py = cdiv(OH, kStPoolH);
+    FCN_REQUIRE(px * py * N < (1ll << 31) && (long long)N * H * W < (1ll << 29), FCN_E_UNSUPPORTED, "stem: problem too large");
+    StemP p;
+    p.x = x; p.w1 = w1; p.b1 = b1; p.w2 = w2; p.b2 = b2; p.y = y;
+    p.H = H; p.W = W; p.CH = CH; p.CW = CW; p.OH = OH; p.OW = OW; p.patches_x = (int)px; p.patches_y = (int)py;
+    p.y_cstride = y_cstride; p.y_coffset = y_coffset; p.relu1 = relu1; p.relu2 = relu2;
+    p.shift = shift; p.alpha_over_n = alpha / 5.f; p.beta = beta; p.kk = lrn_k;
+    const dim3 grid((unsigned)(px * py * N));
+    if (planar)
+        hipLaunchKernelGGL(stem_fwd_kernel<true>, grid, dim3(kStThreads), 0, as_stream(s), p);
+    else
+        hipLaunchKernelGGL(stem_fwd_kernel<false>, grid, dim3(kStThreads), 0, as_stream(s), p);
+    FCN_LAUNCH_CHECK("stem_fwd");
+    return 0;
+}
+
+}
diff --git a/fcn_object_detector_amd/detector.py b/fcn_object_detector_amd/detector.py
--- a/fcn_object_detector_amd/detector.py
+++ b/fcn_object_detector_amd/detector.py
@@ -294,6 +294,7 @@
     def _enqueue_batch(self, dev_ptr: int, layout: Sequence[Tuple[int, int, int]], same: bool) -> None:
         eng = self.engine
         data = eng.blobs["data"]
+        eng.claim_inputs()
         if same:
             L.call("fcn_preprocess_bgr8_batch", dev_ptr, len(layout), layout[0][1], layout[0][2], data.ptr, self._half_flag(data),
                    self.im_height, self.im_width, data.cstride, data.upload_shift, self._minmax_batch_holder[0].ptr, eng.stream)
@@ -326,6 +327,7 @@
             stage[...] = frame.reshape(-1)
             data = eng.blobs["data"]
             L.call("fcn_memcpy_h2d_async", self._frame_dev.ptr, stage.ctypes.data, frame.nbytes, eng.stream)
+            eng.claim_inputs()
             L.call("fcn_preprocess_bgr8_rois", self._frame_dev.ptr, h, w, rects.ctypes.data, len(rects), data.ptr, self._half_flag(data),
                    self.im_height, self.im_width, data.cstride, data.upload_shift, self._minmax.ptr, eng.stream)
             eng.forward_enqueue()
@@ -369,6 +371,7 @@
             stage[...] = frame.reshape(-1)
             data = eng.blobs["data"]
             L.call("fcn_memcpy_h2d_async", self._frame_dev.ptr, stage.ctypes.data, frame.nbytes, eng.stream)
+            eng.claim_inputs()
             L.call("fcn_preprocess_bgr8_rois", self._frame_dev.ptr, h, w, rects.ctypes.data, len(rects), data.ptr, self._half_flag(data),
                    self.im_height, self.im_width, data.cstride, data.upload_shift, self._minmax.ptr, eng.stream)
             eng.forward_enqueue()
@@ -409,6 +412,7 @@
             stage[...] = frame.reshape(-1)
             data = eng.blobs["data"]
             L.call("fcn_memcpy_h2d_async", self._frame_dev.ptr, stage.ctypes.data, frame.nbytes, eng.stream)
+            eng.claim_inputs()
             L.call("fcn_preprocess_bgr8_batch", self._frame_dev.ptr, 1, h, w, data.ptr, self._half_flag(data), self.im_height, self.im_width,
                    data.cstride, data.upload_shift, self._minmax.ptr, eng.stream)
             eng.forward_enqueue()
diff --git a/fcn_object_detector_amd/engine.py b/fcn_object_detector_amd/engine.py
--- a/fcn_object_detector_amd/engine.py
+++ b/fcn_object_detector_amd/engine.py
@@ -305,6 +305,10 @@
 
 
 class Engine:
+
+    _planar_inputs: frozenset = frozenset()
+    _io_pass = False
+    _frame_staged = False
 
     def __init__(self, spec: NetSpec, data_shapes: Optional[Dict[str, Tuple[int, ...]]] = None,
                  params: Optional[Dict[str, List[np.ndarray]]] = None, device: int = 0,
@@ -356,6 +360,9 @@
         self._bn_ws_bytes = 0
         self._bn_ws: Optional[DeviceBuffer] = None
         self._lazy_blob_ops: Dict[str, List[Op]] = {}
+        self._planar_inputs: set = set()
+        self._io_pass = False
+        self._frame_staged = False
         self.loss_blobs: Dict[str, float] = {}
         self.device_fed: set = set()
         self.dropout_seed = 0
@@ -841,6 +848,8 @@
             self._bn_ws = DeviceBuffer(self._bn_ws_bytes, zero=False)
         if self.fuse and self.spec.phase == "TEST" and os.environ.get("FCN_FUSE_POOL_LRN", "1") != "0":
             tasks = self._fuse_pool_lrn(tasks)
+            if not self.f16:
+                tasks = self._fuse_stem(tasks)
         levels = task_levels(tasks, self.group_convs)
         if self.autotune and self.group_convs and self.fuse and not self.f16 and self.spec.phase == "TEST" and os.environ.get("FCN_LEVEL_MOVE", "1") != "0":
             self.tuner.move_floaters(tasks, levels)
@@ -1255,6 +1264,87 @@
             i += 2
         return out
 
+    def _lone_conv_op(self, t: ConvTask) -> Op:
+        lib = L.load()
+        arr, parr = (L.ConvDesc * 1)(t.desc), (L.PoolDesc * 1)()
+        ws = DeviceBuffer(int(lib.fcn_conv2d_group_workspace_bytes(1)), zero=False)
+        self._group_workspaces.append(ws)
+        grp = L.ConvGroup()
+        cfg = self.tuner.conv_cfg(t.layer.name, arr, 1, ws, parr, 0) if self.autotune else -1
+        L.call("fcn_conv2d_group_prepare_fused", arr, 1, parr, 0, ws.ptr, cfg, C.byref(grp))
+        self._keep.extend([arr, parr, ws, grp])
+        op = Op("conv", "%s [cfg%d %dwg]" % (t.layer.name, grp.cfg, grp.total_tiles),
+                lambda st: L.check(lib.fcn_conv2d_fwd_group_f32(C.byref(grp), st)), t.flops, t.bytes)
+        op.cfg = int(grp.cfg)
+        return op
+
+    def _fuse_stem(self, tasks: List[Task]) -> List[Task]:
+        mode = os.environ.get("FCN_STEM_FUSED", "")
+        if mode == "0":
+            return tasks
+        B, lib = self.blobs, L.load()
+        inplace = lambda q: q.type == "ReLU" and q.bottoms == q.tops
+        for i in range(len(tasks) - 1):
+            a, b = tasks[i], tasks[i + 1]
+            fold = getattr(b.ops[0], "fold", None) if isinstance(b, OpTask) and len(b.ops) == 1 else None
+            if not isinstance(a, ConvTask) or fold is None or (mode != "1" and not self.autotune):
+                continue
+            la, lb, ct, ksp, (al, be, kk) = fold
+            l1, d1, d2 = a.layer, a.desc, ct.desc
+            c1, xname = l1.tops[0], l1.bottoms[0]
+            xb = B[xname]
+            if (d1.kh, d1.kw, d1.stride, d1.pad, d1.Cin, d1.x_cstride, d1.Cout) != (7, 7, 2, 3, 4, 4, 64) or (d1.flags & ~L.CONV_RELU) or d1.in_shift != 0.0 \
+                    or d1.y_coffset or d1.y_cstride != 64 or d1.y2 or ksp != (3, 2, 0) or xb.esize != 4 or xb.nchw is None or xb.nchw[1] != 3:
+                continue
+            if la.bottoms != [c1] or [q.name for q in self.consumers.get(c1, []) if not inplace(q)] != [la.name] \
+                    or len([q for q in self.producers.get(c1, []) if not inplace(q)]) != 1 or c1 in self.outputs or c1 in self.alias:
+                continue
+            n, _, h, w = xb.nchw
+            oh, ow = d2.OH, d2.OW
+            relu1, relu2 = (1 if d.flags & L.CONV_RELU else 0 for d in (d1, d2))
+            root, views = xname, [xname]
+            while root in self.alias and self.alias[root][1] == 0 and len(self.consumers.get(self.alias[root][0], [])) == 1:
+                root = self.alias[root][0]
+                views.append(root)
+            rb = B[root]
+            planar = os.environ.get("FCN_STEM_PLANAR", "1") != "0" and rb.is_input and root not in self.alias and not set(views) & set(self.outputs) \
+                and [q.name for q in self.consumers.get(xname, [])] == [l1.name] and not rb.coffset and rb.nchw == xb.nchw and rb.esize == 4
+            stage = None
+
+            def launch(st, from_frame):
+                if from_frame:
+                    L.check(lib.fcn_stem_fwd_f32(stage.ptr, 1, rb.upload_shift, n, h, w, d1.w, d1.bias, relu1, al, be, kk, d2.w, d2.bias, relu2,
+                                                 d2.y, oh, ow, d2.y_cstride, d2.y_coffset, st))
+                else:
+                    L.check(lib.fcn_stem_fwd_f32(d1.x, 0, 0.0, n, h, w, d1.w, d1.bias, relu1, al, be, kk, d2.w, d2.bias, relu2,
+                                                 d2.y, oh, ow, d2.y_cstride, d2.y_coffset, st))
+
+            run = lambda st: launch(st, planar and self._io_pass and root not in self.device_fed)
+            conv_op, fold_op = self._lone_conv_op(a), b.ops[0]
+            if conv_op.cfg != int(lib.fcn_conv2d_first_layer_config()):
+                continue
+            stem_op = Op("stem", "%s+%s" % (l1.name, fold_op.name), run, a.flops + fold_op.flops,
+                         4.0 * (n * h * w * 3 + 64 * 49 * 3 + 64 * 64 + 128 + n * oh * ow * 64))
+            if mode != "1":
+                split = lambda: (conv_op.run(self.stream), fold_op.run(self.stream))
+                if not self.tuner.stem_fused("%s+%s" % (l1.name, fold_op.name), split, lambda: launch(self.stream, False)):
+                    continue
+            stage = self._stage(root) if planar else None
+            for from_frame in ((False, True) if planar else (False,)):
+                launch(self.stream, from_frame)
+            L.call("fcn_stream_sync", self.stream)
+            first: List[Op] = []
+            if planar:
+                self._planar_inputs.add(root)
+                first = [Op("layout", root, lambda st: self._settle_inputs())]
+                for v in views:
+                    self._lazy_blob_ops[v] = first
+            self._lazy_blob_ops[c1] = first + [conv_op]
+            for mid in (la.tops[0], lb.tops[0]):
+                self._lazy_blob_ops[mid] = first + [conv_op] + self._lazy_blob_ops[mid]
+            return tasks[:i] + [OpTask(ct.layer, [stem_op], reads=a.reads, writes=b.writes)] + tasks[i + 2:]
+        return tasks
+
     def _pool_lrn_conv_op(self, la: Layer, lb: Layer, ct: ConvTask) -> Optional[Op]:
         if os.environ.get("FCN_FUSE_POOL_LRN_CONV", "1") == "0" or la.type != "Pooling":
             return None
@@ -1281,9 +1371,11 @@
         al, be, kk = float(lp.get("alpha", 1.0)), float(lp.get("beta", 0.75)), float(lp.get("k", 1.0))
         relu = 1 if d.flags & L.CONV_RELU else 0
         fn = lib.fcn_maxpool_lrn5_conv1x1_fwd_f16 if esz == 2 else lib.fcn_maxpool_lrn5_conv1x1_fwd_f32
-        return Op("pool_lrn_conv", "%s+%s+%s" % (la.name, lb.name, lc.name), lambda st: L.check(fn(
+        op = Op("pool_lrn_conv", "%s+%s+%s" % (la.name, lb.name, lc.name), lambda st: L.check(fn(
             xb.ptr, n, h, w, c, xb.cstride, k, s, pad, oh, ow, al, be, kk, d.w, d.bias, d.Cout, relu, d.y, d.y_cstride, d.y_coffset, st)),
             ct.flops, float(esz) * (xb.pixels * c + n * oh * ow * d.Cout))
+        op.fold = (la, lb, ct, (k, s, pad), (al, be, kk))
+        return op
 
     def _pool_lrn_op(self, la: Layer, lb: Layer) -> Optional[Op]:
         B, lib = self.blobs, L.load()
@@ -1750,9 +1842,9 @@
         dst = b.ptr if b.nchw is None else self._stage(name).ptr
         L.check(L.load().fcn_memcpy_h2d_async(dst, host.ctypes.data, host.nbytes, stream))
 
-    def _upload_convert(self, name: str, stream: Optional[int]) -> None:
+    def _upload_convert(self, name: str, stream: Optional[int], lazy: bool = False) -> None:
         b = self.blobs[name]
-        if b.nchw is None:
+        if b.nchw is None or (name in self._planar_inputs and self._io_pass and not lazy):
             return
         lib = L.load()
         n, c, h, w = b.nchw
@@ -1926,11 +2018,9 @@
                 self._enqueue_targets()
             if self.graph_score is not None:
                 L.call("fcn_graph_launch", self.graph_score, self.stream)
+                self._frame_staged = any(nm not in self.device_fed for nm in self._planar_inputs)
             else:
-                for nm in self.inputs:
-                    if nm not in self.device_fed:
-                        self._upload_convert(nm, self.stream)
-                self.run_ops(self.stream)
+                self._run_ops_uploaded()
             for b in self.blobs.values():
                 b.host_valid = False
             self.score_forwards += 1
@@ -1948,6 +2038,24 @@
             op.run(stream)
 
     def _capture(self, with_io: bool, download: bool = True) -> int:
+        self._io_pass = with_io
+        try:
+            return self._capture_pass(with_io, download)
+        finally:
+            self._io_pass = False
+
+    def _run_ops_uploaded(self) -> None:
+        self._io_pass = True
+        try:
+            for nm in self.inputs:
+                if nm not in self.device_fed:
+                    self._upload_convert(nm, self.stream)
+            self.run_ops(self.stream)
+        finally:
+            self._io_pass = False
+        self._frame_staged = any(nm not in self.device_fed for nm in self._planar_inputs)
+
+    def _capture_pass(self, with_io: bool, download: bool) -> int:
         if with_io:
             for nm in list(self.inputs) + list(self.outputs):
                 self.host_array(nm)
@@ -1987,6 +2095,7 @@
             if nm not in self.device_fed:
                 self._upload_copy(nm, self.stream)
         L.call("fcn_graph_launch", self.graph_io, self.stream)
+        self._frame_staged = any(nm not in self.device_fed for nm in self._planar_inputs)
         for nm in self.outputs:
             self._download_copy(nm, self.stream)
         self._download_counts(self.stream)
@@ -2004,8 +2113,8 @@
             else:
                 for nm in self.inputs:
                     if nm not in self.device_fed:
-                        self._enqueue_upload(nm, self.stream)
-                self.run_ops(self.stream)
+                        self._upload_copy(nm, self.stream)
+                self._run_ops_uploaded()
                 for nm in self.outputs:
                     self._enqueue_download(nm, self.stream)
                 self._download_counts(self.stream)
@@ -2034,8 +2143,8 @@
             else:
                 for nm in self.inputs:
                     if nm not in self.device_fed:
-                        self._enqueue_upload(nm, self.stream)
-                self.run_ops(self.stream)
+                        self._upload_copy(nm, self.stream)
+                self._run_ops_uploaded()
                 for nm in self.outputs:
                     self._enqueue_download(nm, self.stream)
                 self._download_counts(self.stream)
@@ -2061,10 +2170,22 @@
         with self.lock:
             for nm in self.inputs:
                 self._enqueue_upload(nm, self.stream)
+            self._frame_staged = False
             L.call("fcn_stream_sync", self.stream)
+
+    def claim_inputs(self) -> None:
+        self._frame_staged = False
+
+    def _settle_inputs(self) -> None:
+        if self._frame_staged:
+            for nm in self._planar_inputs:
+                if nm not in self.device_fed:
+                    self._upload_convert(nm, self.stream, lazy=True)
+            self._frame_staged = False
 
     def forward_enqueue(self) -> None:
         with self.lock:
+            self._settle_inputs()
             if graphs_enabled():
                 if self.graph_core is None:
                     self.graph_core = self._capture(with_io=False)
@@ -2080,6 +2201,7 @@
         use_graph = use_graph and graphs_enabled()
         with self.lock:
             L.call("fcn_init", self.device)
+            self._settle_inputs()
             if use_graph and self.graph_core is None:
                 self.graph_core = self._capture(with_io=False)
             e0, e1 = C.c_void_p(), C.c_void_p()
@@ -2268,6 +2390,7 @@
 
     def _run_resident(self, engines, iters, lib, time) -> float:
         for e in engines:
+            e._settle_inputs()
             if e.graph_core is None:
                 e.forward_resident(1)
             L.call("fcn_stream_sync", e.stream)
diff --git a/fcn_object_detector_amd/lib.py b/fcn_object_detector_amd/lib.py
--- a/fcn_object_detector_amd/lib.py
+++ b/fcn_object_detector_amd/lib.py
@@ -227,6 +227,7 @@
     "fcn_lrn_fwd_f32": (_i, [_vp, _vp, _vp, _i, _i, _i, _i, _i, _f, _f, _f, _vp]),
     "fcn_maxpool_lrn5_fwd_f32": (_i, [_vp, _vp] + [_i] * 12 + [_f, _f, _f, _vp]),
     "fcn_maxpool_lrn5_fwd_f16": (_i, [_vp, _vp] + [_i] * 12 + [_f, _f, _f, _vp]),
+    "fcn_stem_fwd_f32": (_i, [_vp, _i, _f, _i, _i, _i, _vp, _vp, _i, _f, _f, _f, _vp, _vp, _i, _vp, _i, _i, _i, _i, _vp]),
     "fcn_maxpool_lrn5_conv1x1_fwd_f32": (_i, [_vp] + [_i] * 10 + [_f, _f, _f, _vp, _vp, _i, _i, _vp, _i, _i, _vp]),
     "fcn_maxpool_lrn5_conv1x1_fwd_f16": (_i, [_vp] + [_i] * 10 + [_f, _f, _f, _vp, _vp, _i, _i, _vp, _i, _i, _vp]),
     "fcn_relu_fwd_f32": (_i, [_vp, _vp, _sz, _f, _vp]),
diff --git a/fcn_object_detector_amd/tune.py b/fcn_object_detector_amd/tune.py
--- a/fcn_object_detector_amd/tune.py
+++ b/fcn_object_detector_amd/tune.py
@@ -177,6 +177,17 @@
         return self.choose(self.key(name), self._valid_cfg(int(L.load().fcn_conv2d_num_configs())),
                            lambda: self.time_conv_cfgs(arr, n, ws, parr, npool)[0])
 
+    def stem_fused(self, name: str, split: Callable[[], None], fused: Callable[[], None]) -> bool:
+        forms, sel = (split, fused), [0]
+        cold = self.cold and os.environ.get("FCN_TUNE_COLD", "1") != "0"
+
+        def select(i: int) -> bool:
+            sel[0] = i
+            return True
+
+        return bool(self.choose("stem|" + self.key(name), lambda v: type(v) is int and v in (0, 1),
+                                lambda: self.fastest((0, 1), select, lambda: forms[sel[0]](), COLD if cold else WARM)[0]))
+
     def wgrad_cfgs(self, ops: Sequence["E.Op"]) -> None:
         ncfg = int(L.load().fcn_conv2d_wgrad_num_configs())
         for op in ops:
diff --git a/include/fcnhip.h b/include/fcnhip.h
--- a/include/fcnhip.h
+++ b/include/fcnhip.h
@@ -132,6 +132,9 @@
 int  fcn_maxpool_lrn5_conv1x1_fwd_f16(const void* x, int N, int H, int W, int C, int x_cstride, int k, int stride, int pad,
                                       int OH, int OW, float alpha, float beta, float lrn_k, const void* w, const float* bias,
                                       int Cout, int relu, void* y, int y_cstride, int y_coffset, fcn_stream_t s);
+int  fcn_stem_fwd_f32(const float* x, int planar, float shift, int N, int H, int W, const float* w1, const float* b1, int relu1,
+                      float alpha, float beta, float lrn_k, const float* w2, const float* b2, int relu2, float* y, int OH, int OW,
+                      int y_cstride, int y_coffset, fcn_stream_t s);
 int  fcn_relu_fwd_f32(const float* x, float* y, size_t count, float negative_slope, fcn_stream_t s);
 int  fcn_sigmoid_fwd_f32(const float* x, float* y, size_t count, fcn_stream_t s);
 int  fcn_power_fwd_f32(const float* x, float* y, size_t count, float power, float scale, float shift, fcn_stream_t s);
```

New measurement: 4561 frames/s (median of 5 runs). 1.01x the previous value.
